# mims-harvard/GNNDelete

Hardware: AMD Instinct MI355X
Metric: Del-op train iters/sec (higher is better)
Workload: dtype f32; 1 GPU; synth-collab GCN 2-layer, 5.0% IN edge deletion, full-graph Del step (both_layerwise, mse_mean); num_nodes=235868, in_dim=128, hidden_dim=128, out_dim=64, train_edges_undirected=2122296, df_edges=53057, sdf_edges=1602188, spmm_nnz=1838056, S1=178921, S2=188697, hip_graph=True, matrix_products=fp32 matrix instruction (v_mfma_f32_32x32x2_f32), parallelism=single, ranks_seen=1

## Files before the change

### gnndelete_amd/_lib.py

```python
import ctypes
import os
import re

_HERE = os.path.dirname(os.path.abspath(__file__))
LIB_PATH = os.environ.get('GNNDELETE_HIP_LIB') or os.path.join(_HERE, 'lib', 'libgnndelete_hip.so')
HEADER_PATH = os.path.join(os.path.dirname(_HERE), 'include', 'gnndelete_hip.h')

_i32, _i64, _f32, _f64, _p = ctypes.c_int32, ctypes.c_int64, ctypes.c_float, ctypes.c_double, ctypes.c_void_p

ABI_VERSION = 9

PROTOTYPES = {
    'gd_abi_version': (ctypes.c_int, []),
    'gd_last_error_string': (ctypes.c_char_p, []),
    'gd_build_source_hash': (ctypes.c_char_p, []),
    'gd_matrix_split': (ctypes.c_int, []),
    'gd_set_matrix_split': (ctypes.c_int, [ctypes.c_int]),
    'gd_csr_from_coo_workspace': (_i64, [_i32, _i64]),
    'gd_csr_from_coo': (ctypes.c_int, [_p, _p, _i64, _i32, _p, _p, _p, _p, _p, _i64, _p]),
    'gd_gcn_norm_f32': (ctypes.c_int, [_p, _p, _i32, _p, _p]),
    'gd_spmm_csr_f32': (ctypes.c_int, [_p, _p, _p, _p, _i64, _p, _i64, _p, _f32, _i32, _i32, _p]),
    'gd_spmm_csr_balanced_f32': (ctypes.c_int, [_p, _i32, _p, _i32, _p, _p, _p, _i64, _p, _i64, _p, _f32, _p, _p, _i32,
                                                _i32, _i32, _p, _p]),
    'gd_spmm_csr_onepass_f32': (ctypes.c_int, [_p, _i32, _p, _p, _p, _i64, _p, _i64, _p, _f32, _p, _i32, _i32, _i32, _p, _p]),
    'gd_spmm_csr_onepass_wide_f32': (ctypes.c_int, [_p, _i32, _p, _p, _p, _i64, _p, _i64, _p, _f32, _p, _i32, _i32, _i32, _p, _p]),
    'gd_rows_gemm_wgrad_reduce_f32': (ctypes.c_int, [_p, _i32, _i32, _i32, _p, _i32, _p, _p, _p, _p, _f64, _f64, _f64, _f64, _p]),
    'gd_step_tail_f32': (ctypes.c_int, [_p, _i32, _i32, _i32, _p, _p, _p, _p, _p, _i32, _i32, _i32, _p, _p, _p, _p, _f64, _f64, _f64, _f64,
                                        _p, _i32, _p, _i32, _p, _i32, _p, _p, _p, _p]),
    'gd_step_tail_parts_f32': (ctypes.c_int, [_p, _i32, _i32, _i32, _p, _p, _p, _p, _p, _i32, _i32, _i32, _p, _p, _p, _p, _f64, _f64, _f64, _f64,
                                        _p, _i32, _p, _i32, _p, _i32, _p, _p, _p, _p]),
    'gd_rgcn_conv_f32': (ctypes.c_int, [_p, _p, _p, _p, _p, _p, _i64, _i32, _p, _i32, _i32, _p, _i64, _i32, _i32, _p]),
    'gd_rowpair_loss_f32': (ctypes.c_int, [_i32, _p, _i64, _p, _p, _i64, _p, _i32, _i32, _p, _p, _i64, _p]),
    'gd_random_walk': (ctypes.c_int, [_p, _p, _i32, _p, _i32, _i32, ctypes.c_uint64, _p, _p]),
    'gd_negative_edges': (ctypes.c_int, [_p, _i64, _i64, ctypes.c_uint64, _p, _i64, _p, _i64, _p]),
    'gd_rank_counts_f32': (ctypes.c_int, [_p, _i64, _p, _i64, _p, _p, _p]),
    'gd_subset_rank_workspace': (_i64, [_i64, _i64]),
    'gd_subset_rank_metrics': (ctypes.c_int, [_p, _p, _p, _p, _p, _i64, _i64, _i64, _i64, _i64, _p, _p, _p, _i64, _p]),
    'gd_rgcn_tile_kl': (ctypes.c_int32, [_i32, _i32, _i32, _i32]),
    'gd_rgcn_pack_weight_f32': (ctypes.c_int, [_p, _i32, _i32, _i32, _i32, _i32, _p, _p]),
    'gd_rgcn_wave_covers': (ctypes.c_int32, [_i32, _i32, _i32]),
    'gd_rgcn_wave_conv_f32': (ctypes.c_int, [_p, _i32, _i32, _p, _i32, _p, _p, _p, _p, _i64, _i32, _p, _i32, _p, _i64, _i32, _i32, _i32, _p]),
    'gd_rgcn_tile_conv_f32': (ctypes.c_int, [_p, _p, _p, _p, _p, _p, _p, _i32, _p, _i64, _i32, _p, _i32, _i32, _p, _i64, _i32,
                                             _i32, _p, _p, _i32, _p, _p]),
    'gd_rgcn_mean_f32': (ctypes.c_int, [_p, _p, _p, _i64, _p, _i64, _i32, _i32, _i32, _p]),
    'gd_gat_aggregate_f32': (ctypes.c_int, [_p, _p, _p, _p, _p, _i64, _p, _i64, _p, _p, _f32, _i32, _i32, _p]),
    'gd_gat_aggregate_bwd_f32': (ctypes.c_int, [_p, _p, _p, _p, _p, _p, _p, _p, _p, _i64, _p, _i64, _p, _i64,
                                                _p, _p, _p, _f32, _i32, _i32, _p]),
    'gd_gat_balanced_scratch': (_i64, [_i32, _i32]),
    'gd_gat_aggregate_balanced_f32': (ctypes.c_int, [_p, _i32, _p, _i32, _i32, _p, _p, _p, _p, _i64, _p, _i64, _p, _p, _p,
                                                     _p, _f32, _i32, _i32, _i32, _p]),
    'gd_gat_edge_grads_balanced_f32': (ctypes.c_int, [_p, _i32, _p, _i32, _p, _p, _p, _p, _p, _p, _i64, _p, _i64, _p,
                                                      _p, _p, _p, _f32, _i32, _i32, _p, _p]),
    'gd_row_dots_f32': (ctypes.c_int, [_p, _i64, _i32, _i32, _p, _p, _p, _p, _p]),
    'gd_gat_transpose_edges_f32': (ctypes.c_int, [_p, _p, _p, _i32, _p, _p, _p]),
    'gd_rank1_add2_f32': (ctypes.c_int, [_p, _i64, _i32, _i32, _p, _p, _p, _p, _p]),
    'gd_segment_sum_f32': (ctypes.c_int, [_p, _p, _p, _i32, _p, _p]),
    'gd_rows_gemm_f32': (ctypes.c_int, [_p, _i64, _p, _i32, _p, _i32, _i32, _i32, _p, _i32, _p, _i64, _p, _p]),
    'gd_rows_gather_gemm_f32': (ctypes.c_int, [_p, _i64, _i64, _p, _i32, _p, _i32, _i32, _p, _i32, _p, _i64, _p]),
    'gd_rows_gemm_wgrad_workspace': (_i64, [_i32, _i32, _i32]),
    'gd_rows_gemm_ws_covers': (ctypes.c_int, [_i32, _i32, _i32]),
    'gd_rows_gemm_accumulate_f32': (ctypes.c_int, [_p, _i64, _p, _i32, _p, _i32, _i32, _i32, _p, _i64, _p]),
    'gd_rows_gemm_select_f32': (ctypes.c_int, [_p, _p, _p, _i64, _p, _i32, _p, _i32, _i32, _i32, _p, _i32, _p, _i64, _p]),
    'gd_rows_gemm_dots_f32': (ctypes.c_int, [_p, _p, _p, _i64, _p, _i32, _i32, _i32, _p, _i32, _p, _i64, _p, _i32, _p, _p, _p, _p,
                                             _p]),
    'gd_rows_gemm_signs_f32': (ctypes.c_int, [_p, _i64, _p, _i32, _p, _i32, _i32, _i32, _p, _i32, _p, _i64, _p, _p, _p]),
    'gd_rows_gemm_gated_f32': (ctypes.c_int, [_p, _i64, _p, _i32, _p, _i32, _i32, _i32, _p, _p, _i64, _p]),
    'gd_gate_rows_f32': (ctypes.c_int, [_p, _i64, _p, _i32, _p, _i32, _p, _i64, _p]),
    'gd_rows_gemm_gated_rank1_f32': (ctypes.c_int, [_p, _i64, _p, _i32, _p, _i32, _i32, _i32, _p, _p, _p, _p, _p, _p, _i64, _p]),
    'gd_rows_gemm_wgrad_f32': (ctypes.c_int, [_p, _i64, _p, _p, _i64, _p, _p, _p, _i32, _i32, _i32, _p, _i32, _p, _p]),
    'gd_induced_subgraph_workspace': (_i64, [_i32]),
    'gd_induced_subgraph': (ctypes.c_int, [_p, _p, _p, _i32, _p, _i32, _p, _i32, _p, _i64, _p, _p, _p, _p, _p, _p, _p, _p, _p,
                                           _p, _i64, _p]),
    'gd_batch_csr_workspace': (_i64, [_i32, _i64]),
    'gd_batch_csr': (ctypes.c_int, [_p, _p, _i64, _i32, _i32, _p, _p, _p, _p, _p, _p, _p, _p, _i64, _p]),
    'gd_batch_loss_terms_workspace': (_i64, [_i32, _i64]),
    'gd_batch_loss_terms': (ctypes.c_int, [_p, _i64, _p, _i64, _i32, _p, _i32, _i32, _f32, _f32, _p, _p, _p, _p, _p, _i64, _p]),
    'gd_rowpair_mse_workspace': (_i64, [_i32]),
    'gd_rowpair_mse_f32': (ctypes.c_int, [_p, _i64, _p, _i64, _i32, _p, _p, _i32, _p, _p, _p, _p, _i64, _i32,
                                          _p, _p, _p]),
    'gd_rowtarget_mse_workspace': (_i64, [_i32]),
    'gd_rowtarget_mse_f32': (ctypes.c_int, [_p, _i64, _p, _i32, _p, _p, _p, _p, _i32, _p, _i64, _p, _p, _p]),
    'gd_rowtarget_mse_pair_covers': (ctypes.c_int32, [_i32, _i32]),
    'gd_rowtarget_mse_pair_f32': (ctypes.c_int, [_p, _i64, _p, _i32, _p, _p, _p, _p, _i32, _p, _i64, _p, _p, _i64, _p, _i32, _p, _p, _p, _p, _i32, _p, _i64, _p, _p]),
    'gd_gemm_f32_workspace': (_i64, [_i32, _i32, _i32]),
    'gd_gemm_f32': (ctypes.c_int, [_p, _i64, _p, _i32, _p, _i32, _i32, _p, _p, _i64, _p, _p]),
    'gd_edge_dot_f32': (ctypes.c_int, [_p, _i64, _i32, _p, _p, _p, _i64, _p, _i64, _p, _p]),
    'gd_edge_dot_bwd_f32': (ctypes.c_int, [_p, _i64, _i32, _p, _p, _p, _i64, _p, _p, _i64, _p, _i64, _p]),
    'gd_rows_gemm_wgrad_adam_f32': (ctypes.c_int, [_p, _i64, _p, _p, _i64, _p, _p, _p, _i32, _i32, _i32, _p, _i32, _p,
                                                   _p, _p, _p, _p, _f64, _f64, _f64, _f64, _p]),
    'gd_rows_gemm_wgrad_blocks': (_i32, [_i32]),
    'gd_rows_gemm_wgrad_loss_f32': (ctypes.c_int, [_p, _i64, _p, _p, _i64, _p, _p, _p, _p, _p, _p, _i32, _i32, _i32, _p, _i32,
                                                   _p, _p, _p, _p, _p, _p, _f64, _f64, _f64, _f64, _p]),
    'gd_del_loss_bwd_blocks': (_i32, [_i32]),
    'gd_del_loss_bwd_f32': (ctypes.c_int, [_p, _i64, _p, _i32, _p, _i32, _p, _p, _p, _p, _p, _i64, _p, _i64, _p, _p]),
    'gd_del_loss_bwd_wgrad_f32': (ctypes.c_int, [_p, _i64, _p, _i32, _p, _i32, _p, _p, _p, _p, _p, _i64, _p, _i64, _p, _p, _p]),
    'gd_del_loss_bwd_wgrad_parts': (ctypes.c_int32, [_i32, _i32]),
    'gd_del_loss_bwd_wgrad_parts_f32': (ctypes.c_int, [_p, _i64, _p, _i32, _p, _i32, _p, _p, _p, _p, _p, _i64, _p, _i64, _p, _p, _i32, _p]),
    'gd_del_loss_fold_wgrad_covers': (ctypes.c_int32, [_i32, _i32, _i32]),
    'gd_del_loss_fold_wgrad_parts_f32': (ctypes.c_int, [_p, _i64, _p, _i32, _p, _i32, _p, _p, _p, _p, _p, _i64, _p, _i32, _p, _p, _p, _i32, _p]),
    'gd_del1_loss_wgrad_covers': (ctypes.c_int32, [_i32, _i32]),
    'gd_del1_loss_wgrad_parts': (ctypes.c_int32, [_i32]),
    'gd_del1_chain_loss_wgrad_f32': (ctypes.c_int, [_p, _i64, _p, _i32, _p, _i32, _p, _i64, _p, _p, _p, _p, _p, _p, _i64, _i32, _p, _p, _p, _p, _p, _p, _p, _i32, _p]),
    'gd_del1_loss_wgrad_f32': (ctypes.c_int, [_p, _i64, _p, _i32, _p, _i32, _p, _i64, _p, _p, _p, _p, _p, _p, _i64, _p, _p, _i32, _p]),
    'gd_rowtarget_mse_blocks': (_i32, [_i32]),
    'gd_rowfold_loss_blocks': (_i32, [_i32]),
    'gd_rowfold_loss_f32': (ctypes.c_int, [_i32, _p, _i64, _p, _i32, _i32, _p, _p, _p, _p, _i32, _p, _i64, _p, _p]),
    'gd_rowfold_kld_scale_f32': (ctypes.c_int, [_p, _i32, _f32, _f32, _f32, _f32, _p, _p, _i32, _i32, _p, _i64, _p, _p]),
    'gd_loss_finalize_f32': (ctypes.c_int, [_p, _i32, _p, _i32, _p, _p, _i32, _p, _p, _p]),
    'gd_pairs_sigmoid_mse_workspace': (_i64, [_i32, _i32]),
    'gd_pairs_sigmoid_mse_f32': (ctypes.c_int, [_p, _i64, _p, _i32, _i32, _p, _i64, _f32, _p, _p, _p, _p]),
    'gd_edgeprob_dec_workspace': (_i64, [_i64, _i32]),
    'gd_edgeprob_dec_f32': (ctypes.c_int, [_p, _i64, _i64, _i32, _p, _i64, _p, _i64, _i64, _f32, _p, _p, _p, _p, _p, _p, _p]),
    'gd_edge_incidence_workspace': (_i64, [_i64, _i64]),
    'gd_edge_incidence': (ctypes.c_int, [_p, _p, _i64, _i64, _p, _p, _p, _p, _i64, _p]),
    'gd_edge_incidence_fixed_bytes': (_i64, [_i64, _i64]),
    'gd_edge_incidence_fixed': (ctypes.c_int, [_p, _p, _i64, _i64, _p, _i64, _p, _i64, _p]),
    'gd_edge_incidence_update_workspace': (_i64, [_i64, _i64]),
    'gd_edge_incidence_update': (ctypes.c_int, [_p, _p, _p, _i64, _i64, _i64, _p, _p, _p, _p, _i64, _p]),
    'gd_rows_add_f32': (ctypes.c_int, [_p, _i64, _i64, _p, _i32, _p, _i64, _f32, _i32, _p]),
    'gd_edgeprob_record_f32': (ctypes.c_int, [_p, _p, _f32, _f32, _p, _i32, _p, _p]),
    'gd_edgeprob_batch_loss_workspace': (_i64, [_i64, _i64, _i32]),
    'gd_edgeprob_batch_loss_f32': (ctypes.c_int, [_p, _i64, _i64, _p, _i64, _i64, _i32, _p, _i64, _p, _i64, _i64, _p, _p, _i64, _f32, _f32,
                                                  _p, _i64, _p, _p, _p, _p, _p, _p, _p, _i64, _p, _p]),
    'gd_edge_bce_workspace': (_i64, [_i64, _i32]),
    'gd_edge_bce_f32': (ctypes.c_int, [_p, _i64, _i64, _i32, _p, _i64, _i64, _p, _i64, _i64, _f32, _p, _p, _p, _p, _p, _p, _p]),
    'gd_col_sum_workspace': (_i64, [_i64, _i32]),
    'gd_col_sum_f32': (ctypes.c_int, [_p, _i64, _i64, _i32, _p, _p, _p, _p, _p, _p]),
    'gd_row_nll_workspace': (_i64, [_i64, _i32]),
    'gd_row_nll_f32': (ctypes.c_int, [_p, _i64, _i64, _i32, _i32, _p, _i64, _p, _f32, _p, _i64, _p, _p, _p]),
    'gd_adam_at_f32': (ctypes.c_int, [_p, _p, _p, _p, _p, _i64, _f64, _f64, _f64, _f64, _p]),
    'gd_adam_f32': (ctypes.c_int, [_p, _p, _p, _p, _p, _i64, _f64, _f64, _f64, _f64, _p]),
    'gd_segment_softmax_f32': (ctypes.c_int, [_p, _p, _i32, _p, _p]),
    'gd_segment_softmax_bwd_f32': (ctypes.c_int, [_p, _p, _p, _i32, _p, _p]),
    'gd_rowpair_dot_f32': (ctypes.c_int, [_p, _i64, _p, _p, _i64, _p, _i64, _i32, _p, _p]),
    'gd_spmm_csr_onepass_aux_f32': (ctypes.c_int, [_p, _i32, _p, _p, _p, _p, _i64, _p, _i64, _p, _i32, _i32, _i32, _p, _p]),
    'gd_typed_wgrad_f32': (ctypes.c_int, [_p, _i32, _p, _p, _p, _p, _i64, _p, _i64, _i32, _i32, _i32, _p, _p]),
    'gd_typed_edge_dot_f32': (ctypes.c_int, [_p, _p, _p, _i64, _p, _i64, _p, _i64, _p, _i32, _i32, _i32, _p, _p]),
    'gd_comm_unique_id': (ctypes.c_int, [_p]),
    'gd_comm_init': (ctypes.c_int, [_p, _i32, _i32, ctypes.POINTER(ctypes.c_void_p)]),
    'gd_comm_destroy': (ctypes.c_int, [_p]),
    'gd_allreduce_f32': (ctypes.c_int, [_p, _i64, _p, _p]),
    'gd_exchange_rows_f32': (ctypes.c_int, [_p, _p, _p, _p, _i32, _i32, _p, _p]),
}

_lib = None


class GnnDeleteHipError(RuntimeError):
    pass


def declared_symbols():
    with open(HEADER_PATH) as f:
        text = re.sub(r'/\*.*?\*/', '', f.read(), flags=re.S)
    return sorted(set(re.findall(r'\b(gd_[a-z0-9_]+)\s*\(', text)))


def _sources_hash():
    from .source_hash import source_files, source_hash
    return source_hash() if all(os.path.exists(f) for f in source_files()) and os.path.isdir(os.path.join(_HERE, 'csrc')) else None


def build_stamp():
    return lib().gd_build_source_hash().decode(), _sources_hash()


def lib():
    global _lib
    if _lib is None:
        if not os.path.exists(LIB_PATH):
            raise GnnDeleteHipError(
                f'{LIB_PATH} is missing: the HIP extension is not built. Run '
                '`python -c "import __graft_entry__ as g; g.build()"` (or `make -C gnndelete_amd/csrc`). '
                'There is no CPU fallback.')
        import torch
        handle = ctypes.CDLL(LIB_PATH)
        for name, (res, args) in PROTOTYPES.items():
            fn = getattr(handle, name)
            fn.restype, fn.argtypes = res, args
        if handle.gd_abi_version() != ABI_VERSION:
            raise GnnDeleteHipError(f'libgnndelete_hip.so ABI version {handle.gd_abi_version()}, this package binds version {ABI_VERSION}: rebuild (make -C gnndelete_amd/csrc)')
        built, here = handle.gd_build_source_hash().decode(), _sources_hash()
        if here is not None and built != here and not os.environ.get('GNNDELETE_HIP_LIB') and os.environ.get('GD_ALLOW_STALE_LIB') != '1':
            raise GnnDeleteHipError(f'{LIB_PATH} was built from other sources (stamp {built}, sources here {here}): run '
                                    '`make -C gnndelete_amd/csrc` (or set GD_ALLOW_STALE_LIB=1 to load it anyway)')
# ... 18 lines not shown
```

### gnndelete_amd/csrc/del_fused.hip

```cpp
#include <stdlib.h>

#include "common.h"

namespace gd {

using f32x16 = __attribute__((ext_vector_type(16))) float;

struct DelLoss {
  const int32_t* slot;
  const float* tm;
  const float* coef;
  const float* cnt_signed;
  float* partials;
};

template <int NT, bool WG>
__global__ __launch_bounds__(256, (NT == 2 && WG) ? 1 : 2) void del_loss_bwd_kernel(const float* __restrict__ p, int64_t ld_p,
                                                              const int32_t* __restrict__ idx, int32_t n_sel,
                                                              const float* __restrict__ w, DelLoss loss,
                                                              float* __restrict__ dz, int64_t ld_dz,
                                                              float* __restrict__ dp, int64_t ld_dp,
                                                              float* __restrict__ wg_partials) {
  constexpr int D = 32 * NT;
  constexpr int PB = D + 4;
// ... 497 lines not shown
#pragma unroll
      for (int i = 0; i < 8; ++i)
        *reinterpret_cast<float4*>(tp + r * PTP + kq * 32 + 4 * i) = make_float4(livef * x[i].x, livef * x[i].y, livef * x[i].z, livef * x[i].w);
      const float cf = ls_cur >= 0 ? cf_raw : 0.f, cn = ls_cur >= 0 ? cn_raw : 0.f;
      float sq = 0.f;
      uint32_t bits[2] = {0u, 0u};
      float* zrow = z + (int64_t)row * ld_z + cb + 4 * kq;
#pragma unroll
      for (int t = 0; t < 4; ++t) {
        const float4 zv = make_float4(acc[t][0], acc[t][1], acc[t][2], acc[t][3]);
        *reinterpret_cast<float4*>(zrow + 16 * t) = zv;
        bits[t >> 1] |= ((zv.x > 0.f ? 1u : 0u) | (zv.y > 0.f ? 2u : 0u) | (zv.z > 0.f ? 4u : 0u) | (zv.w > 0.f ? 8u : 0u)) << (16 * (t & 1) + 4 * kq);
        const float4 d4 = make_float4(zv.x - tv[t].x, zv.y - tv[t].y, zv.z - tv[t].z, zv.w - tv[t].w);
        sq = fmaf(d4.x, d4.x, sq); sq = fmaf(d4.y, d4.y, sq); sq = fmaf(d4.z, d4.z, sq); sq = fmaf(d4.w, d4.w, sq);
        float4 gv = make_float4(cf * d4.x, cf * d4.y, cf * d4.z, cf * d4.w);
        if (HAS_ADD) gv = f4_add(gv, av[t]);
        *reinterpret_cast<float4*>(tz + r * PTZ + 16 * t + 4 * kq) = gv;
      }
      sq *= livef;
      if (cn >= 0.f) ls0 = fmaf(cn, sq, ls0); else ls1 = fmaf(-cn, sq, ls1);
#pragma unroll
      for (int q = 0; q < 2; ++q) {
        bits[q] |= (uint32_t)__shfl_xor((int)bits[q], 16);
        bits[q] |= (uint32_t)__shfl_xor((int)bits[q], 32);
      }
      if (live && kq == 0) {
        sign_out[(int64_t)s_a * 4 + 2 * half + 0] = bits[0];
        sign_out[(int64_t)s_a * 4 + 2 * half + 1] = bits[1];
      }
      __builtin_amdgcn_sched_barrier(0);
      fetch_rows(row_n);
      fetch_targets(ls_n, row_n);
      __builtin_amdgcn_fence(__ATOMIC_ACQ_REL, "wavefront");
      __builtin_amdgcn_wave_barrier();
#pragma unroll
      for (int sp = 0; sp < 4; ++sp) {
        float a_op[8], b_op[4];
#pragma unroll
        for (int ta = 0; ta < 8; ++ta) a_op[ta] = tp[(4 * sp + kq) * PTP + 16 * ta + r];
#pragma unroll
        for (int tb = 0; tb < 4; ++tb) b_op[tb] = tz[(4 * sp + kq) * PTZ + 16 * tb + r];
#pragma unroll
        for (int ta = 0; ta < 8; ++ta)
#pragma unroll
          for (int tb = 0; tb < 4; ++tb)
            gacc[ta * 4 + tb] = __builtin_amdgcn_mfma_f32_16x16x4f32(a_op[ta], b_op[tb], gacc[ta * 4 + tb], 0, 0, 0);
      }
      __builtin_amdgcn_fence(__ATOMIC_ACQ_REL, "wavefront");
      __builtin_amdgcn_wave_barrier();
      __builtin_amdgcn_sched_barrier(0);
    }
  }
  __syncthreads();
  float* const red = wl;
#pragma unroll
  for (int ta = 0; ta < 8; ++ta)
#pragma unroll
    for (int tb = 0; tb < 4; ++tb)
#pragma unroll
      for (int v = 0; v < 4; ++v) red[wave * D * H + (16 * ta + 4 * kq + v) * H + 16 * tb + r] = gacc[ta * 4 + tb][v];
  __syncthreads();
  for (int slot = blockIdx.x; slot < n_part; slot += gridDim.x) {
    float* const out = wg_partials + (int64_t)slot * D * D;
    const bool mine = slot == (int)blockIdx.x;
    for (int e = tid; e < D * D; e += 256) {
      const int i = e >> 7, c = e & 127, hf = c >> 6, ch = c & 63;
      out[e] = mine ? red[hf * D * H + i * H + ch] + red[(2 + hf) * D * H + i * H + ch] : 0.f;
    }
  }
  ls0 = wave_sum(ls0);
  ls1 = wave_sum(ls1);
  if (lane == 0) { lred[0][wave] = ls0; lred[1][wave] = ls1; }
  __syncthreads();
  if (tid == 0) {
    for (int slot = blockIdx.x; slot < n_part; slot += gridDim.x) {
      const bool mine = slot == (int)blockIdx.x;
      loss.partials[2 * slot + 0] = mine ? (lred[0][0] + lred[0][1]) + (lred[0][2] + lred[0][3]) : 0.f;
      loss.partials[2 * slot + 1] = mine ? (lred[1][0] + lred[1][1]) + (lred[1][2] + lred[1][3]) : 0.f;
    }
  }
}

struct ChainRank1 { const float* ra; const float* ua; const float* rb; const float* ub; };
template <bool RANK1>
__global__ __launch_bounds__(256) __attribute__((amdgpu_waves_per_eu(1, 1))) void del1_chain_ws_kernel(
    const float* __restrict__ p, int64_t ld_p, const int32_t* __restrict__ idx, int32_t n_sel, const float* __restrict__ w,
    float* __restrict__ z, int64_t ld_z, uint32_t* __restrict__ sign_io, DelLoss loss, const float* __restrict__ dt, int64_t ld_dt,
    const float* __restrict__ w_next, float* __restrict__ wg_partials, int32_t n_part, ChainRank1 r1) {
  constexpr int D = 128, H = 64, PTP = 144, PTZ = 80;
  constexpr int kTiles = 4 * (16 * PTP + 16 * PTZ);
  extern __shared__ __attribute__((aligned(16))) float wl[];
  __shared__ float lred[2][4];
  const int tid = threadIdx.x, lane = tid & 63;
  const int wave = __builtin_amdgcn_readfirstlane(tid >> 6);
  const int half = wave & 1, pair = wave >> 1, cb = H * half;
  const int r = lane & 15, kq = lane >> 4;
  float* const tp = wl + wave * (16 * PTP + 16 * PTZ);
  float* const tz = tp + 16 * PTP;
  float4* const wimg = reinterpret_cast<float4*>(wl + kTiles);
  float4* const w2img = wimg + 2 * 4 * 8 * 64;
  {
    float4 fv[16];
#pragma unroll
    for (int it = 0; it < 16; ++it) {
      const int e = tid + 256 * it;
      const int ln = e & 63, i_ = (e >> 6) & 7, t_ = (e >> 9) & 3, h_ = e >> 11;
      const float* src = w + (int64_t)(16 * i_ + 4 * (ln >> 4)) * D + 64 * h_ + 16 * t_ + (ln & 15);
      fv[it] = make_float4(src[0], src[D], src[2 * D], src[3 * D]);
    }
#pragma unroll
    for (int it = 0; it < 16; ++it) wimg[tid + 256 * it] = fv[it];
#pragma unroll
    for (int it = 0; it < 8; ++it) {
      const int e = tid + 256 * it;
      const int ln = e & 63, i_ = (e >> 6) & 3, t_ = (e >> 8) & 3, h_ = e >> 10;
      const float* src = w_next + (int64_t)(16 * i_ + 4 * (ln >> 4)) * D + 64 * h_ + 16 * t_ + (ln & 15);
      fv[it] = make_float4(src[0], src[D], src[2 * D], src[3 * D]);
    }
#pragma unroll
    for (int it = 0; it < 8; ++it) w2img[tid + 256 * it] = fv[it];
  }
  __syncthreads();
  const float4* const wmine = wimg + (half * 4) * 8 * 64 + lane;
  const float4* const w2mine = w2img + (half * 4) * 4 * 64 + lane;
  const int n_units = (n_sel + 15) >> 4;
  const int n_pairs = gridDim.x * 2, pid = blockIdx.x * 2 + pair;
  const int u_lo = (int)((int64_t)n_units * pid / n_pairs), u_hi = (int)((int64_t)n_units * (pid + 1) / n_pairs);

  auto slot_of = [&](int u) -> int { return min(min(u, n_units - 1) * 16 + r, n_sel - 1); };
  int32_t row_n = idx[slot_of(u_lo)], ls_n = loss.slot[slot_of(u_lo)];
  int32_t row_nn = idx[slot_of(u_lo + 1)], ls_nn = loss.slot[slot_of(u_lo + 1)];
  __builtin_amdgcn_sched_barrier(0);
  f32x4w gacc[32];
#pragma unroll
  for (int i = 0; i < 32; ++i) gacc[i] = f32x4w{0.f, 0.f, 0.f, 0.f};
  float ls0 = 0.f, ls1 = 0.f;

  float4 x[8], dv[4], tv[4];
  float4 ua4[RANK1 ? 4 : 1], ub4[RANK1 ? 4 : 1];
  float ra_row = 0.f, rb_row = 0.f;
  if (RANK1) {
#pragma unroll
    for (int t = 0; t < 4; ++t) {
      ua4[t] = *reinterpret_cast<const float4*>(r1.ua + cb + 16 * t + 4 * kq);
      ub4[t] = *reinterpret_cast<const float4*>(r1.ub + cb + 16 * t + 4 * kq);
    }
  }
  uint2 old_bits;
  float cf_raw, cn_raw;
  int32_t ls_cur;
  auto fetch_targets = [&](int32_t u) {
    const int uc = max(u, 0);
    const float* trow = loss.tm + (int64_t)uc * D + cb + 4 * kq;
#pragma unroll
    for (int t = 0; t < 4; ++t) tv[t] = *reinterpret_cast<const float4*>(trow + 16 * t);
    cf_raw = loss.coef[uc];
    cn_raw = loss.cnt_signed[uc];
    ls_cur = u;
  };
  auto fetch_rows = [&](int32_t row, int u) {
    const float4* src = reinterpret_cast<const float4*>(p + (int64_t)row * ld_p + 4 * kq);
#pragma unroll
    for (int i = 0; i < 8; ++i) x[i] = src[4 * i];
    const float4* dsrc = reinterpret_cast<const float4*>(dt + (int64_t)row * ld_dt + 4 * kq);
#pragma unroll
    for (int i = 0; i < 4; ++i) dv[i] = dsrc[4 * i];
    old_bits = *reinterpret_cast<const uint2*>(sign_io + (int64_t)slot_of(u) * 4 + 2 * half);
    if (RANK1) { ra_row = r1.ra[row]; rb_row = r1.rb[row]; }
  };
  if (u_lo < u_hi) {
    fetch_rows(row_n, u_lo);
    fetch_targets(ls_n);
    for (int u = u_lo; u < u_hi; ++u) {
      const int32_t row = row_n;
      const int s_a = min(u, n_units - 1) * 16 + r;
      const bool live = s_a < n_sel;
      const float livef = live ? 1.f : 0.f;
      row_n = row_nn;
      ls_n = ls_nn;
      row_nn = idx[slot_of(u + 2)];
      ls_nn = loss.slot[slot_of(u + 2)];
      f32x4w acc[4], dacc[4];
      {
        float4 wq[2][4];
#pragma unroll
        for (int t = 0; t < 4; ++t) wq[0][t] = wmine[(t * 8) * 64];
#pragma unroll
        for (int i = 0; i < 8; ++i) {
          if (i + 1 < 8) {
#pragma unroll
            for (int t = 0; t < 4; ++t) wq[(i + 1) & 1][t] = wmine[(t * 8 + i + 1) * 64];
          }
          const float xv[4] = {x[i].x, x[i].y, x[i].z, x[i].w};
#pragma unroll
          for (int c = 0; c < 4; ++c)
#pragma unroll
            for (int t = 0; t < 4; ++t) {
              const float4 wf = wq[i & 1][t];
              const float wa = c == 0 ? wf.x : c == 1 ? wf.y : c == 2 ? wf.z : wf.w;
              if (i == 0 && c == 0) acc[t] = __builtin_amdgcn_mfma_f32_16x16x4f32(wa, xv[0], f32x4w{0.f, 0.f, 0.f, 0.f}, 0, 0, 0);
              else acc[t] = __builtin_amdgcn_mfma_f32_16x16x4f32(wa, xv[c], acc[t], 0, 0, 0);
            }
        }
#pragma unroll
        for (int t = 0; t < 4; ++t) wq[0][t] = w2mine[(t * 4) * 64];
#pragma unroll
        for (int i = 0; i < 4; ++i) {
          if (i + 1 < 4) {
#pragma unroll
            for (int t = 0; t < 4; ++t) wq[(i + 1) & 1][t] = w2mine[(t * 4 + i + 1) * 64];
          }
          const float xv[4] = {dv[i].x, dv[i].y, dv[i].z, dv[i].w};
#pragma unroll
          for (int c = 0; c < 4; ++c)
#pragma unroll
            for (int t = 0; t < 4; ++t) {
              const float4 wf = wq[i & 1][t];
              const float wa = c == 0 ? wf.x : c == 1 ? wf.y : c == 2 ? wf.z : wf.w;
              if (i == 0 && c == 0) dacc[t] = __builtin_amdgcn_mfma_f32_16x16x4f32(wa, xv[0], f32x4w{0.f, 0.f, 0.f, 0.f}, 0, 0, 0);
              else dacc[t] = __builtin_amdgcn_mfma_f32_16x16x4f32(wa, xv[c], dacc[t], 0, 0, 0);
            }
        }
      }
      __builtin_amdgcn_sched_barrier(0);
#pragma unroll
      for (int i = 0; i < 8; ++i)
        *reinterpret_cast<float4*>(tp + r * PTP + 16 * i + 4 * kq) = make_float4(livef * x[i].x, livef * x[i].y, livef * x[i].z, livef * x[i].w);
      const float cf = ls_cur >= 0 ? cf_raw : 0.f, cn = ls_cur >= 0 ? cn_raw : 0.f;
      float sq = 0.f;
      uint32_t bits[2] = {0u, 0u};
      const uint32_t ob[2] = {old_bits.x, old_bits.y};
      const float ra_c = ra_row, rb_c = rb_row;
      float* zrow = z + (int64_t)row * ld_z + cb + 4 * kq;
#pragma unroll
      for (int t = 0; t < 4; ++t) {
        const float4 zv = make_float4(acc[t][0], acc[t][1], acc[t][2], acc[t][3]);
        *reinterpret_cast<float4*>(zrow + 16 * t) = zv;
        bits[t >> 1] |= ((zv.x > 0.f ? 1u : 0u) | (zv.y > 0.f ? 2u : 0u) | (zv.z > 0.f ? 4u : 0u) | (zv.w > 0.f ? 8u : 0u)) << (16 * (t & 1) + 4 * kq);
        const float4 d4 = make_float4(zv.x - tv[t].x, zv.y - tv[t].y, zv.z - tv[t].z, zv.w - tv[t].w);
        sq = fmaf(d4.x, d4.x, sq); sq = fmaf(d4.y, d4.y, sq); sq = fmaf(d4.z, d4.z, sq); sq = fmaf(d4.w, d4.w, sq);
        const uint32_t m = ob[t >> 1] >> (16 * (t & 1) + 4 * kq);
        float4 dq = make_float4(dacc[t][0], dacc[t][1], dacc[t][2], dacc[t][3]);
        if (RANK1) {
          dq.x = fmaf(rb_c, ub4[t].x, fmaf(ra_c, ua4[t].x, dq.x)); dq.y = fmaf(rb_c, ub4[t].y, fmaf(ra_c, ua4[t].y, dq.y));
          dq.z = fmaf(rb_c, ub4[t].z, fmaf(ra_c, ua4[t].z, dq.z)); dq.w = fmaf(rb_c, ub4[t].w, fmaf(ra_c, ua4[t].w, dq.w));
        }
        const float4 gv = make_float4(cf * d4.x + ((m & 1u) ? dq.x : 0.f), cf * d4.y + ((m & 2u) ? dq.y : 0.f),
                                      cf * d4.z + ((m & 4u) ? dq.z : 0.f), cf * d4.w + ((m & 8u) ? dq.w : 0.f));
        *reinterpret_cast<float4*>(tz + r * PTZ + 16 * t + 4 * kq) = gv;
      }
      sq *= livef;
      if (cn >= 0.f) ls0 = fmaf(cn, sq, ls0); else ls1 = fmaf(-cn, sq, ls1);
#pragma unroll
      for (int q = 0; q < 2; ++q) {
        bits[q] |= (uint32_t)__shfl_xor((int)bits[q], 16);
        bits[q] |= (uint32_t)__shfl_xor((int)bits[q], 32);
      }
      if (live && kq == 0) *reinterpret_cast<uint2*>(sign_io + (int64_t)s_a * 4 + 2 * half) = make_uint2(bits[0], bits[1]);
      __builtin_amdgcn_sched_barrier(0);
      fetch_rows(row_n, u + 1);
      fetch_targets(ls_n);
      __builtin_amdgcn_fence(__ATOMIC_ACQ_REL, "wavefront");
      __builtin_amdgcn_wave_barrier();
#pragma unroll
      for (int sp = 0; sp < 4; ++sp) {
        float a_op[8], b_op[4];
#pragma unroll
        for (int ta = 0; ta < 8; ++ta) a_op[ta] = tp[(4 * sp + kq) * PTP + 16 * ta + r];
#pragma unroll
        for (int tb = 0; tb < 4; ++tb) b_op[tb] = tz[(4 * sp + kq) * PTZ + 16 * tb + r];
#pragma unroll
        for (int ta = 0; ta < 8; ++ta)
#pragma unroll
          for (int tb = 0; tb < 4; ++tb)
            gacc[ta * 4 + tb] = __builtin_amdgcn_mfma_f32_16x16x4f32(a_op[ta], b_op[tb], gacc[ta * 4 + tb], 0, 0, 0);
      }
      __builtin_amdgcn_fence(__ATOMIC_ACQ_REL, "wavefront");
      __builtin_amdgcn_wave_barrier();
      __builtin_amdgcn_sched_barrier(0);
    }
  }
  __syncthreads();
  float* const red = wl;
#pragma unroll
  for (int ta = 0; ta < 8; ++ta)
#pragma unroll
    for (int tb = 0; tb < 4; ++tb)
#pragma unroll
      for (int v = 0; v < 4; ++v) red[wave * D * H + (16 * ta + 4 * kq + v) * H + 16 * tb + r] = gacc[ta * 4 + tb][v];
  __syncthreads();
  for (int slot = blockIdx.x; slot < n_part; slot += gridDim.x) {
    float* const out = wg_partials + (int64_t)slot * D * D;
    const bool mine = slot == (int)blockIdx.x;
    for (int e = tid; e < D * D; e += 256) {
      const int i = e >> 7, c = e & 127, hf = c >> 6, ch = c & 63;
      out[e] = mine ? red[hf * D * H + i * H + ch] + red[(2 + hf) * D * H + i * H + ch] : 0.f;
    }
  }
  ls0 = wave_sum(ls0);
  ls1 = wave_sum(ls1);
  if (lane == 0) { lred[0][wave] = ls0; lred[1][wave] = ls1; }
  __syncthreads();
  if (tid == 0) {
    for (int slot = blockIdx.x; slot < n_part; slot += gridDim.x) {
      const bool mine = slot == (int)blockIdx.x;
      loss.partials[2 * slot + 0] = mine ? (lred[0][0] + lred[0][1]) + (lred[0][2] + lred[0][3]) : 0.f;
      loss.partials[2 * slot + 1] = mine ? (lred[1][0] + lred[1][1]) + (lred[1][2] + lred[1][3]) : 0.f;
    }
  }
}

static inline int del_fused_grid(int32_t n_sel) {
  const int n_tiles = (n_sel + 31) / 32;
  int grid = (n_tiles + 3) / 4;
  if (grid > 1024) grid = 1024;
  return grid < 1 ? 1 : grid;
}

}

extern "C" int32_t gd_del_loss_bwd_blocks(int32_t n_sel) { return n_sel > 0 ? gd::del_fused_grid(n_sel) : 0; }

extern "C" int32_t gd_rows_gemm_wgrad_blocks(int32_t n_sel);

static int del_loss_bwd_impl(const float* p, int64_t ld_p, const int32_t* idx, int32_t n_sel, const float* w,
                             int32_t d, const int32_t* loss_slot, const float* tm, const float* coef,
                             const float* cnt_signed, float* dz, int64_t ld_dz, float* dp, int64_t ld_dp,
                             float* loss_partials, float* wgrad_partials, bool with_wgrad, void* stream, int32_t n_part_req = 0) {
  using namespace gd;
  const char* name = with_wgrad ? "gd_del_loss_bwd_wgrad_f32" : "gd_del_loss_bwd_f32";
  if (n_sel == 0) return GD_OK;
  GD_REQUIRE(p && idx && w && loss_slot && tm && coef && cnt_signed && dp && loss_partials && (with_wgrad ? wgrad_partials != nullptr : dz != nullptr),
             GD_E_NULL, "%s: null pointer", name);
  GD_REQUIRE(d == 32 || d == 64, GD_E_DIM, "%s: d=%d must be 32 or 64", name, d);
  GD_REQUIRE(ld_p >= d && (!dz || ld_dz >= d) && ld_dp >= d && ld_p % 4 == 0 && (!dz || ld_dz % 4 == 0) && ld_dp % 4 == 0, GD_E_DIM,
             "%s: bad row strides", name);
  GD_REQUIRE(aligned16(p) && aligned16(tm) && (!dz || aligned16(dz)) && aligned16(dp) && (!with_wgrad || aligned16(wgrad_partials)), GD_E_ALIGN,
             "%s: unaligned", name);
  GD_REQUIRE(p != dp && p != dz && dz != dp, GD_E_DIM, "%s: buffers must not alias", name);
  hipStream_t s = (hipStream_t)stream;
  const DelLoss loss{loss_slot, tm, coef, cnt_signed, loss_partials};
  if (!with_wgrad) {
    const dim3 grid(del_fused_grid(n_sel));
    const size_t lds = ((size_t)d * d + (size_t)d * (d + 4)) * sizeof(float);
    switch (d / 32) {
      case 1: hipLaunchKernelGGL((del_loss_bwd_kernel<1, false>), grid, dim3(256), lds, s, p, ld_p, idx, n_sel, w, loss, dz, ld_dz, dp, ld_dp, nullptr); break;
      default: hipLaunchKernelGGL((del_loss_bwd_kernel<2, false>), grid, dim3(256), lds, s, p, ld_p, idx, n_sel, w, loss, dz, ld_dz, dp, ld_dp, nullptr); break;
    }
    return launched("del_loss_bwd");
  }
  static const bool ws_on = [] { const char* e = getenv("GD_DEL2_WS"); return !(e && atoi(e) == 0); }();
  if (ws_on && d == 64 && n_sel >= 65536) {
    const int n_all = gd_rows_gemm_wgrad_blocks(n_sel);
    const int n_part = n_part_req > 0 ? n_part_req : n_all;
    GD_REQUIRE(n_part <= n_all && n_part >= (ws_cu_count() < n_all ? ws_cu_count() : n_all), GD_E_DIM,
               "%s: n_part=%d outside [gd_del_loss_bwd_wgrad_parts, gd_rows_gemm_wgrad_blocks = %d]", name, n_part, n_all);
    const int grid_ws = ws_cu_count() < n_part ? ws_cu_count() : n_part;
    constexpr int kLdsWs = 4 * 64 * 64 * 4;
    if (dz) {
      static const hipError_t a1 = hipFuncSetAttribute(reinterpret_cast<const void*>(&del_loss_bwd_ws_kernel<true>), hipFuncAttributeMaxDynamicSharedMemorySize, kLdsWs);
      if (a1 != hipSuccess) return fail(-(int)a1, "gd_del_loss_bwd_wgrad_f32: %s", hipGetErrorString(a1));
      hipLaunchKernelGGL((del_loss_bwd_ws_kernel<true>), dim3(grid_ws), dim3(256), kLdsWs, s, p, ld_p, idx, n_sel, w, loss, dz, ld_dz, dp, ld_dp,
                         wgrad_partials, n_part, DelFold{nullptr, nullptr});
    } else {
      static const hipError_t a0 = hipFuncSetAttribute(reinterpret_cast<const void*>(&del_loss_bwd_ws_kernel<false>), hipFuncAttributeMaxDynamicSharedMemorySize, kLdsWs);
      if (a0 != hipSuccess) return fail(-(int)a0, "gd_del_loss_bwd_wgrad_f32: %s", hipGetErrorString(a0));
      hipLaunchKernelGGL((del_loss_bwd_ws_kernel<false>), dim3(grid_ws), dim3(256), kLdsWs, s, p, ld_p, idx, n_sel, w, loss, dz, ld_dz, dp, ld_dp,
                         wgrad_partials, n_part, DelFold{nullptr, nullptr});
    }
    return launched("del_loss_bwd_ws");
  }
  GD_REQUIRE(n_part_req == 0 || n_part_req == gd_rows_gemm_wgrad_blocks(n_sel), GD_E_DIM,
             "%s: n_part=%d but this size leaves gd_rows_gemm_wgrad_blocks(n_sel) = %d partials", name, n_part_req, gd_rows_gemm_wgrad_blocks(n_sel));
  const dim3 grid(gd_rows_gemm_wgrad_blocks(n_sel));
#define GD_DF_CASE(NT_)                                                                                                        \
  do {                                                                                                                         \
    constexpr int kD = 32 * NT_;                                                                                               \
    constexpr int kLds = (kD * kD + kD * (kD + 4) + 4 * 32 * (kD + 4)) * 4;                                                    \
    static_assert(kLds >= 4 * kD * kD * 4, "block sum needs 4 D^2 floats");                                                    \
// ... 68 lines not shown
  static const hipError_t at = hipFuncSetAttribute(reinterpret_cast<const void*>(&del_loss_bwd_ws_kernel<false, true>), hipFuncAttributeMaxDynamicSharedMemorySize, kLdsWs);
  if (at != hipSuccess) return fail(-(int)at, "%s: %s", name, hipGetErrorString(at));
  const DelLoss loss{loss_slot, tm, coef, cnt_signed, loss_partials};
  hipLaunchKernelGGL((del_loss_bwd_ws_kernel<false, true>), dim3(grid_ws), dim3(256), kLdsWs, (hipStream_t)stream, p, ld_p, idx, n_sel, w, loss,
                     static_cast<float*>(nullptr), (int64_t)0, g, ld_g, wgrad_partials, n_part, DelFold{w_next, w_fold});
  return launched("del_loss_fold_ws");
}

extern "C" int32_t gd_del1_loss_wgrad_covers(int32_t n_sel, int32_t d) {
  static const bool on = [] { const char* e = getenv("GD_DEL1_FUSED"); return !(e && atoi(e) == 0); }();
  return on && d == 128 && n_sel >= 65536 ? 1 : 0;
}

extern "C" int32_t gd_del1_loss_wgrad_parts(int32_t n_sel) {
  if (n_sel <= 0) return 0;
  const int nb = gd_rows_gemm_wgrad_blocks(n_sel);
  return gd::ws_cu_count() < nb ? gd::ws_cu_count() : nb;
}

extern "C" int gd_del1_loss_wgrad_f32(const float* p, int64_t ld_p, const int32_t* idx, int32_t n_sel, const float* w, int32_t d,
                                      float* z, int64_t ld_z, uint32_t* sign_out, const int32_t* loss_slot, const float* tm,
                                      const float* coef, const float* cnt_signed, const float* g_add, int64_t ld_gadd,
                                      float* loss_partials, float* wgrad_partials, int32_t n_part, void* stream) {
  using namespace gd;
  const char* name = "gd_del1_loss_wgrad_f32";
  if (n_sel == 0) return GD_OK;
  GD_REQUIRE(p && idx && w && z && sign_out && loss_slot && tm && coef && cnt_signed && loss_partials && wgrad_partials, GD_E_NULL,
             "%s: null pointer", name);
  GD_REQUIRE(d == 128, GD_E_DIM, "%s: d=%d must be 128 (other widths: gd_rows_gemm_signs_f32 + gd_rows_gemm_wgrad_loss_f32)", name, d);
  GD_REQUIRE(ld_p >= d && ld_z >= d && ld_p % 4 == 0 && ld_z % 4 == 0 && (!g_add || (ld_gadd >= d && ld_gadd % 4 == 0)), GD_E_DIM,
             "%s: bad row strides", name);
  GD_REQUIRE(aligned16(p) && aligned16(z) && aligned16(tm) && aligned16(w) && (!g_add || aligned16(g_add)) && aligned16(wgrad_partials),
             GD_E_ALIGN, "%s: unaligned", name);
  GD_REQUIRE(p != z && g_add != z, GD_E_DIM, "%s: z must not alias p or g_add (the two waves of a pair read whole rows)", name);
  hipStream_t s = (hipStream_t)stream;
  const DelLoss loss{loss_slot, tm, coef, cnt_signed, loss_partials};
  GD_REQUIRE(n_part >= 1 && n_part <= gd_rows_gemm_wgrad_blocks(n_sel), GD_E_DIM,
             "%s: n_part=%d outside [1, gd_rows_gemm_wgrad_blocks(n_sel)=%d]", name, n_part, gd_rows_gemm_wgrad_blocks(n_sel));
  const int grid = ws_cu_count() < n_part ? ws_cu_count() : n_part;
  constexpr int kLds = 4 * 128 * 64 * 4;
  if (g_add) {
    static const hipError_t a1 = hipFuncSetAttribute(reinterpret_cast<const void*>(&del1_loss_wgrad_ws_kernel<true>), hipFuncAttributeMaxDynamicSharedMemorySize, kLds);
    if (a1 != hipSuccess) return fail(-(int)a1, "%s: %s", name, hipGetErrorString(a1));
    hipLaunchKernelGGL((del1_loss_wgrad_ws_kernel<true>), dim3(grid), dim3(256), kLds, s, p, ld_p, idx, n_sel, w, z, ld_z, sign_out, loss, g_add,
                       ld_gadd, wgrad_partials, n_part);
  } else {
    static const hipError_t a0 = hipFuncSetAttribute(reinterpret_cast<const void*>(&del1_loss_wgrad_ws_kernel<false>), hipFuncAttributeMaxDynamicSharedMemorySize, kLds);
    if (a0 != hipSuccess) return fail(-(int)a0, "%s: %s", name, hipGetErrorString(a0));
    hipLaunchKernelGGL((del1_loss_wgrad_ws_kernel<false>), dim3(grid), dim3(256), kLds, s, p, ld_p, idx, n_sel, w, z, ld_z, sign_out, loss, nullptr,
                       0, wgrad_partials, n_part);
  }
  return launched("del1_loss_wgrad_ws");
}

extern "C" int gd_del1_chain_loss_wgrad_f32(const float* p, int64_t ld_p, const int32_t* idx, int32_t n_sel, const float* w, int32_t d,
                                            float* z, int64_t ld_z, uint32_t* sign_io, const int32_t* loss_slot, const float* tm,
                                            const float* coef, const float* cnt_signed, const float* dt, int64_t ld_dt, int32_t d_next,
                                            const float* w_next, const float* row_a, const float* col_a, const float* row_b,
                                            const float* col_b, float* loss_partials, float* wgrad_partials, int32_t n_part,
                                            void* stream) {
  using namespace gd;
  const char* name = "gd_del1_chain_loss_wgrad_f32";
  if (n_sel == 0) return GD_OK;
  GD_REQUIRE(p && idx && w && z && sign_io && loss_slot && tm && coef && cnt_signed && dt && w_next && loss_partials && wgrad_partials, GD_E_NULL,
             "%s: null pointer", name);
  GD_REQUIRE(d == 128 && d_next == 64, GD_E_DIM, "%s: widths %d / %d must be 128 / 64", name, d, d_next);
  GD_REQUIRE(ld_p >= d && ld_z >= d && ld_dt >= d_next && ld_p % 4 == 0 && ld_z % 4 == 0 && ld_dt % 4 == 0, GD_E_DIM, "%s: bad row strides", name);
  GD_REQUIRE(aligned16(p) && aligned16(z) && aligned16(tm) && aligned16(dt) && aligned16(wgrad_partials) && (reinterpret_cast<uintptr_t>(sign_io) & 7u) == 0,
             GD_E_ALIGN, "%s: unaligned", name);
  GD_REQUIRE(p != z && dt != z, GD_E_DIM, "%s: z must not alias p or dt", name);
  GD_REQUIRE(n_part >= 1 && n_part <= gd_rows_gemm_wgrad_blocks(n_sel), GD_E_DIM,
             "%s: n_part=%d outside [1, gd_rows_gemm_wgrad_blocks(n_sel)=%d]", name, n_part, gd_rows_gemm_wgrad_blocks(n_sel));
  const DelLoss loss{loss_slot, tm, coef, cnt_signed, loss_partials};
  const int grid = ws_cu_count() < n_part ? ws_cu_count() : n_part;
  constexpr int kLds = (4 * (16 * 144 + 16 * 80) + 128 * 128 + 64 * 128) * 4;
  const bool rank1 = row_a || col_a || row_b || col_b;
  GD_REQUIRE(!rank1 || (row_a && col_a && row_b && col_b && aligned16(col_a) && aligned16(col_b)), GD_E_NULL,
             "%s: the rank-1 terms come as four pointers (row_a, col_a, row_b, col_b; 16-byte aligned column vectors)", name);
  const ChainRank1 r1{row_a, col_a, row_b, col_b};
  if (rank1) {
    static const hipError_t at = hipFuncSetAttribute(reinterpret_cast<const void*>(&del1_chain_ws_kernel<true>), hipFuncAttributeMaxDynamicSharedMemorySize, kLds);
    if (at != hipSuccess) return fail(-(int)at, "%s: %s", name, hipGetErrorString(at));
    hipLaunchKernelGGL(del1_chain_ws_kernel<true>, dim3(grid), dim3(256), kLds, (hipStream_t)stream, p, ld_p, idx, n_sel, w, z, ld_z, sign_io, loss, dt,
                       ld_dt, w_next, wgrad_partials, n_part, r1);
  } else {
    static const hipError_t at = hipFuncSetAttribute(reinterpret_cast<const void*>(&del1_chain_ws_kernel<false>), hipFuncAttributeMaxDynamicSharedMemorySize, kLds);
    if (at != hipSuccess) return fail(-(int)at, "%s: %s", name, hipGetErrorString(at));
    hipLaunchKernelGGL(del1_chain_ws_kernel<false>, dim3(grid), dim3(256), kLds, (hipStream_t)stream, p, ld_p, idx, n_sel, w, z, ld_z, sign_io, loss, dt,
                       ld_dt, w_next, wgrad_partials, n_part, r1);
  }
  return launched("del1_chain_ws");
}
```

### gnndelete_amd/csrc/rows_gemm.hip

```cpp
#include "common.h"

namespace gd {

using f32x16 = __attribute__((ext_vector_type(16))) float;
using bf16x8 = __attribute__((ext_vector_type(8))) __bf16;
using bf16x2 = __attribute__((ext_vector_type(2))) __bf16;
using f32x2 = __attribute__((ext_vector_type(2))) float;
using u32x4v = __attribute__((ext_vector_type(4))) uint32_t;

__device__ inline void split8(const float4 a, const float4 b, bf16x8 (&s)[3]) {
  const f32x2 v[4] = {{a.x, a.y}, {a.z, a.w}, {b.x, b.y}, {b.z, b.w}};
  u32x4v p[3];
#pragma unroll
  for (int i = 0; i < 4; ++i) {
    f32x2 r = v[i];
#pragma unroll
    for (int q = 0; q < 3; ++q) {
      const uint32_t w = __builtin_bit_cast(uint32_t, __builtin_convertvector(r, bf16x2));
      p[q][i] = w;
      if (q < 2) {
        f32x2 h;
        h[0] = __builtin_bit_cast(float, w << 16);
        h[1] = __builtin_bit_cast(float, w & 0xffff0000u);
        r = r - h;
// ... 567 lines not shown
  }
}

__global__ __launch_bounds__(256) void wgrad_reduce_kernel(const float* __restrict__ partials, int32_t n_part,
                                                           int32_t n_elem, int32_t accumulate,
                                                           float* __restrict__ dw) {
  __shared__ float4 red[16][16];
  const int v = threadIdx.x & 15, slice = threadIdx.x >> 4;
  const int e4 = blockIdx.x * 16 + v;
  const int n4 = n_elem >> 2;
  float4 s0 = f4_zero(), s1 = f4_zero(), s2 = f4_zero(), s3 = f4_zero();
  if (e4 < n4) {
    int b = slice;
    for (; b + 48 < n_part; b += 64) {
      const float4 p0 = reinterpret_cast<const float4*>(partials + (int64_t)b * n_elem)[e4];
      const float4 p1 = reinterpret_cast<const float4*>(partials + (int64_t)(b + 16) * n_elem)[e4];
      const float4 p2 = reinterpret_cast<const float4*>(partials + (int64_t)(b + 32) * n_elem)[e4];
      const float4 p3 = reinterpret_cast<const float4*>(partials + (int64_t)(b + 48) * n_elem)[e4];
      s0 = f4_add(s0, p0); s1 = f4_add(s1, p1); s2 = f4_add(s2, p2); s3 = f4_add(s3, p3);
    }
    for (; b < n_part; b += 16) s0 = f4_add(s0, reinterpret_cast<const float4*>(partials + (int64_t)b * n_elem)[e4]);
  }
  red[slice][v] = f4_add(f4_add(s0, s1), f4_add(s2, s3));
  __syncthreads();
  if (slice == 0 && e4 < n4) {
    float4 t = accumulate ? reinterpret_cast<float4*>(dw)[e4] : f4_zero();
#pragma unroll
    for (int i = 0; i < 16; ++i) t = f4_add(t, red[i][v]);
    reinterpret_cast<float4*>(dw)[e4] = t;
  }
}

__global__ __launch_bounds__(256) void wgrad_reduce_adam_kernel(const float* __restrict__ partials, int32_t n_part,
                                                                int32_t n_elem, int32_t accumulate,
                                                                float* __restrict__ dw, float* __restrict__ param,
                                                                float* __restrict__ m, float* __restrict__ v,
                                                                const int32_t* __restrict__ iter, double lr, double beta1,
                                                                double beta2, double eps) {
  __shared__ float4 red[16][16];
  const int vv = threadIdx.x & 15, slice = threadIdx.x >> 4;
  const int e4 = blockIdx.x * 16 + vv;
  const int n4 = n_elem >> 2;
  float4 s0 = f4_zero(), s1 = f4_zero(), s2 = f4_zero(), s3 = f4_zero();
  if (e4 < n4) {
    int b = slice;
    for (; b + 48 < n_part; b += 64) {
      const float4 p0 = reinterpret_cast<const float4*>(partials + (int64_t)b * n_elem)[e4];
      const float4 p1 = reinterpret_cast<const float4*>(partials + (int64_t)(b + 16) * n_elem)[e4];
      const float4 p2 = reinterpret_cast<const float4*>(partials + (int64_t)(b + 32) * n_elem)[e4];
      const float4 p3 = reinterpret_cast<const float4*>(partials + (int64_t)(b + 48) * n_elem)[e4];
      s0 = f4_add(s0, p0); s1 = f4_add(s1, p1); s2 = f4_add(s2, p2); s3 = f4_add(s3, p3);
    }
    for (; b < n_part; b += 16) s0 = f4_add(s0, reinterpret_cast<const float4*>(partials + (int64_t)b * n_elem)[e4]);
  }
  red[slice][vv] = f4_add(f4_add(s0, s1), f4_add(s2, s3));
  __syncthreads();
  if (slice == 0 && e4 < n4) {
    float4 t4 = accumulate ? reinterpret_cast<float4*>(dw)[e4] : f4_zero();
#pragma unroll
    for (int i = 0; i < 16; ++i) t4 = f4_add(t4, red[i][vv]);
    reinterpret_cast<float4*>(dw)[e4] = t4;
    const AdamScalars sc = adam_scalars(lr, beta1, beta2, eps, *iter + 1);
    float4 p4 = reinterpret_cast<float4*>(param)[e4], m4 = reinterpret_cast<float4*>(m)[e4],
           v4 = reinterpret_cast<float4*>(v)[e4];
    adam_update(p4.x, m4.x, v4.x, t4.x, sc);
    adam_update(p4.y, m4.y, v4.y, t4.y, sc);
    adam_update(p4.z, m4.z, v4.z, t4.z, sc);
    adam_update(p4.w, m4.w, v4.w, t4.w, sc);
    reinterpret_cast<float4*>(param)[e4] = p4;
    reinterpret_cast<float4*>(m)[e4] = m4;
    reinterpret_cast<float4*>(v)[e4] = v4;
  }
}

struct TailJob {
  const float* partials; int32_t n_part, n_elem, accumulate;
  float* dw; float* param; float* m; float* v;
};
struct TailFin {
  const float* p1; int32_t n1; const float* p2; int32_t n2;
  float* hist; int32_t capacity; int32_t* pos; int32_t* iter; int32_t* arrive;
};

__global__ __launch_bounds__(256) void step_tail_kernel(TailJob j1, TailJob j2, TailFin fin, double lr, double beta1, double beta2,
                                                        double eps) {
  __shared__ float4 red[16][16];
  __shared__ float fred[4][256];
  __shared__ int32_t t_sh;
  const int nb1 = (j1.n_elem / 4 + 15) / 16, nb2 = (j2.n_elem / 4 + 15) / 16;
  const int tid = threadIdx.x;
  if ((int)blockIdx.x < nb1 + nb2) {
    const bool first = (int)blockIdx.x < nb1;
    const TailJob j = first ? j1 : j2;
    const int blk = first ? blockIdx.x : blockIdx.x - nb1;
    if (tid == 0) {
      int32_t t = atomicAdd(fin.iter, 0);
      asm volatile("" : "+v"(t));
      atomicAdd(fin.arrive + (t < 0 ? 1 : 0), 1);
      t_sh = t + 1;
    }
    const int vv = tid & 15, slice = tid >> 4;
    const int e4 = blk * 16 + vv;
    const int n4 = j.n_elem >> 2;
    float4 s0 = f4_zero(), s1 = f4_zero(), s2 = f4_zero(), s3 = f4_zero();
    if (e4 < n4) {
      int b = slice;
      for (; b + 48 < j.n_part; b += 64) {
        const float4 p0 = reinterpret_cast<const float4*>(j.partials + (int64_t)b * j.n_elem)[e4];
        const float4 p1 = reinterpret_cast<const float4*>(j.partials + (int64_t)(b + 16) * j.n_elem)[e4];
        const float4 p2 = reinterpret_cast<const float4*>(j.partials + (int64_t)(b + 32) * j.n_elem)[e4];
        const float4 p3 = reinterpret_cast<const float4*>(j.partials + (int64_t)(b + 48) * j.n_elem)[e4];
        s0 = f4_add(s0, p0); s1 = f4_add(s1, p1); s2 = f4_add(s2, p2); s3 = f4_add(s3, p3);
      }
      for (; b < j.n_part; b += 16) s0 = f4_add(s0, reinterpret_cast<const float4*>(j.partials + (int64_t)b * j.n_elem)[e4]);
    }
    red[slice][vv] = f4_add(f4_add(s0, s1), f4_add(s2, s3));
    __syncthreads();
    if (slice == 0 && e4 < n4) {
      float4 t4 = j.accumulate ? reinterpret_cast<float4*>(j.dw)[e4] : f4_zero();
#pragma unroll
      for (int i = 0; i < 16; ++i) t4 = f4_add(t4, red[i][vv]);
      reinterpret_cast<float4*>(j.dw)[e4] = t4;
      const AdamScalars sc = adam_scalars(lr, beta1, beta2, eps, t_sh);
      float4 p4 = reinterpret_cast<float4*>(j.param)[e4], m4 = reinterpret_cast<float4*>(j.m)[e4],
             v4 = reinterpret_cast<float4*>(j.v)[e4];
      adam_update(p4.x, m4.x, v4.x, t4.x, sc);
      adam_update(p4.y, m4.y, v4.y, t4.y, sc);
      adam_update(p4.z, m4.z, v4.z, t4.z, sc);
      adam_update(p4.w, m4.w, v4.w, t4.w, sc);
      reinterpret_cast<float4*>(j.param)[e4] = p4;
      reinterpret_cast<float4*>(j.m)[e4] = m4;
      reinterpret_cast<float4*>(j.v)[e4] = v4;
    }
    return;
  }
  float a = 0.f, b = 0.f, c = 0.f, d = 0.f;
  for (int i = tid; i < fin.n1; i += 256) { a += fin.p1[2 * i]; b += fin.p1[2 * i + 1]; }
  for (int i = tid; i < fin.n2; i += 256) { c += fin.p2[2 * i]; d += fin.p2[2 * i + 1]; }
  fred[0][tid] = a; fred[1][tid] = b; fred[2][tid] = c; fred[3][tid] = d;
  __syncthreads();
  for (int off = 128; off > 0; off >>= 1) {
    if (tid < off) {
#pragma unroll
      for (int q = 0; q < 4; ++q) fred[q][tid] += fred[q][tid + off];
    }
    __syncthreads();
  }
  if (tid < 4) fin.hist[(int64_t)(*fin.pos) * 4 + tid] = fred[tid][0];
  __syncthreads();
  if (tid == 0) {
    while (atomicAdd(fin.arrive, 0) < nb1 + nb2) __builtin_amdgcn_s_sleep(8);
    *fin.arrive = 0;
    *fin.pos = (*fin.pos + 1) % fin.capacity;
    atomicAdd(fin.iter, 1);
  }
}

__global__ __launch_bounds__(256) void wgrad_reduce_scalar_kernel(const float* __restrict__ partials, int32_t n_part,
                                                                  int32_t n_elem, int32_t accumulate,
                                                                  float* __restrict__ dw) {
  const int e = blockIdx.x * 256 + threadIdx.x;
  if (e >= n_elem) return;
  float s = accumulate ? dw[e] : 0.f;
  for (int b = 0; b < n_part; ++b) s += partials[(int64_t)b * n_elem + e];
  dw[e] = s;
}

static inline void wgrad_geometry(int32_t n_sel, int* n_blocks, int* rows_per_block) {
  int nb = (n_sel + 127) / 128;
  if (nb > 512) nb = 512;
  if (nb < (n_sel + kWgradMaxRows - 1) / kWgradMaxRows) nb = (n_sel + kWgradMaxRows - 1) / kWgradMaxRows;
  if (nb < 1) nb = 1;
  int rpb = (n_sel + nb - 1) / nb;
  rpb = (rpb + 31) / 32 * 32;
  if (rpb < 32) rpb = 32;
  *n_blocks = (n_sel + rpb - 1) / rpb;
  if (*n_blocks < 1) *n_blocks = 1;
  *rows_per_block = rpb;
}

}

static int rows_gemm_impl(const float* in, int64_t ld_in, const int32_t* idx, int32_t n_sel, const float* w,
                          int32_t d_in, int32_t d_out, int32_t trans_w, const float* bias, int32_t relu_in,
                          const uint32_t* gate_bits, uint32_t* sign_out, float* out, int64_t ld_out,
                          float* save_in, void* stream, const float* in_alt = nullptr, const uint8_t* sel = nullptr,
                          gd::RowDots dots = gd::RowDots{nullptr, nullptr, nullptr, nullptr}, const int64_t* gidx = nullptr,
                          int32_t n_in = 0) {
  using namespace gd;
  GD_REQUIRE(!sel || (in_alt && aligned16(in_alt) && in_alt != out && !gate_bits && !sign_out), GD_E_NULL,
             "gd_rows_gemm_select_f32: bad in_alt");
  GD_REQUIRE(in && w && out, GD_E_NULL, "gd_rows_gemm_f32: null pointer");
  GD_REQUIRE(n_sel >= 0 && d_in > 0 && d_out > 0 && ld_in >= d_in && ld_out >= d_out, GD_E_DIM,
             "gd_rows_gemm_f32: bad dims n_sel=%d d_in=%d d_out=%d", n_sel, d_in, d_out);
  GD_REQUIRE(in != out || d_in == d_out, GD_E_DIM, "gd_rows_gemm_f32: in-place needs d_in == d_out");
  GD_REQUIRE(!(gate_bits && sign_out), GD_E_DIM, "gd_rows_gemm_f32: gate and sign output are exclusive");
  if (n_sel == 0) return GD_OK;
  if (!gidx) {
    const int rc = rows_gemm_ws_try(in, ld_in, idx, n_sel, w, d_in, d_out, trans_w, bias, relu_in, gate_bits, sign_out, out, ld_out,
                                    save_in, stream, in_alt, sel, dots.u1, dots.u2, dots.o1, dots.o2);
    if (rc != 1) return rc;
  }
  hipStream_t s = (hipStream_t)stream;
  size_t lds = (size_t)d_in * 32 * (d_out / 32 == 3 ? 4 : d_out / 32) * sizeof(float);
  const int np = matrix_split();
  const bool mfma_ok = (d_out % 32 == 0) && d_out <= 128 && (d_in % 32 == 0) && lds <= 64 * 1024 && aligned16(in) &&
                       (ld_in % 4 == 0) && (!save_in || aligned16(save_in)) && aligned16(out) && (ld_out % 4 == 0) &&
                       (!bias || aligned16(bias));
  if (mfma_ok) {
    const int n_tiles = (n_sel + 31) / 32;
    int grid = (n_tiles + 7) / 8;
    static const int grid_cap = [] { const char* e = getenv("GD_ROWS_GEMM_GRID"); return e && atoi(e) > 0 ? atoi(e) : 512; }();
    if (grid > grid_cap) grid = grid_cap;
    static const bool spread_on = [] { const char* e = getenv("GD_ROWS_GEMM_SPREAD"); return !(e && atoi(e) == 0); }();
    if (spread_on && grid < ws_cu_count()) grid = n_tiles < ws_cu_count() ? n_tiles : ws_cu_count();
    const int kc_split = (np && (d_in == 64 || d_in == 128) && d_out >= 96) ? d_in / 32 : 0;
    const bool narrow_split = np && !kc_split && d_out == 64 && d_in == 128;
    if (kc_split || narrow_split) {
      lds = (size_t)3 * d_in * d_out * 2;
      if (grid > grid_cap / 2 && lds > 80 * 1024) grid = grid_cap / 2;
    }
    static const bool queue_on = [] { const char* e = getenv("GD_ROWS_GEMM_QUEUE"); return !(e && atoi(e) == 0); }();
    const bool use_queue = queue_on && !kc_split && !narrow_split && n_tiles >= 16 * 256 && !gidx;
    if (use_queue && grid > ws_cu_count()) grid = ws_cu_count();
#define GD_RG_KERNEL(NT, MODE, SELV, NPV, KCV, GV)                                                                 \
  do {                                                                                                            \
    if (use_queue && !NPV && !GV) {                                                                                 \
      auto kq = rows_gemm_mfma_kernel<NT, MODE, SELV, 0, 0, true>;                                                \
              \
      static const hipError_t onceq = hipFuncSetAttribute((const void*)kq, hipFuncAttributeMaxDynamicSharedMemorySize, 64 * 1024 + 64); \
      GD_REQUIRE(onceq == hipSuccess, -(int)onceq, "gd_rows_gemm_f32: cannot raise the LDS limit of the tile-queue kernel"); \
      hipLaunchKernelGGL(kq, dim3(grid), dim3(1024), lds, s, in, ld_in, idx, n_sel, w, d_in, trans_w,             \
                         bias, relu_in, out, ld_out, save_in, gate_bits, sign_out, in_alt, sel, dots, gidx, n_in); \
      break;                                                                                                      \
    }                                                                                                             \
    auto kern = rows_gemm_mfma_kernel<NT, MODE, SELV, NPV, KCV, false, GV>;                                            \
    if (NPV && lds > 64 * 1024) {                                                                                 \
      static const hipError_t once = hipFuncSetAttribute((const void*)kern, hipFuncAttributeMaxDynamicSharedMemorySize, 160 * 1024); \
// ... 199 lines not shown
  return gd_adam_at_f32(adam->param, dw, adam->m, adam->v, adam->iter, n_elem, adam->lr, adam->beta1, adam->beta2,
                        adam->eps, stream);
}

extern "C" int gd_rows_gemm_wgrad_f32(const float* a, int64_t ld_a, const int32_t* a_idx, const float* g, int64_t ld_g,
                                      const int32_t* g_idx, const float* relu_mask, const float* g_add,
                                      int32_t n_sel, int32_t d_a, int32_t d_b, float* dw, int32_t accumulate,
                                      float* partials, void* stream) {
  return wgrad_impl(nullptr, a, ld_a, a_idx, g, ld_g, g_idx, relu_mask, g_add, n_sel, d_a, d_b, dw, accumulate,
                    partials, nullptr, stream);
}

extern "C" int gd_rows_gemm_wgrad_adam_f32(const float* a, int64_t ld_a, const int32_t* a_idx, const float* g,
                                           int64_t ld_g, const int32_t* g_idx, const float* relu_mask,
                                           const float* g_add, int32_t n_sel, int32_t d_a, int32_t d_b, float* dw,
                                           int32_t accumulate, float* partials,
                                           float* param, float* exp_avg, float* exp_avg_sq, const int32_t* iter,
                                           double lr, double beta1, double beta2, double eps, void* stream) {
  GD_REQUIRE(param && exp_avg && exp_avg_sq && iter, GD_E_NULL, "gd_rows_gemm_wgrad_adam_f32: null optimizer state");
  const gd::AdamArgs adam{param, exp_avg, exp_avg_sq, iter, lr, beta1, beta2, eps};
  return wgrad_impl(nullptr, a, ld_a, a_idx, g, ld_g, g_idx, relu_mask, g_add, n_sel, d_a, d_b, dw, accumulate,
                    partials, &adam, stream);
}

extern "C" int gd_rows_gemm_wgrad_reduce_f32(const float* partials, int32_t n_sel, int32_t d_a, int32_t d_b, float* dw,
                                             int32_t accumulate, float* param, float* exp_avg, float* exp_avg_sq,
                                             const int32_t* iter, double lr, double beta1, double beta2, double eps,
                                             void* stream) {
  GD_REQUIRE(partials && dw, GD_E_NULL, "gd_rows_gemm_wgrad_reduce_f32: null pointer");
  GD_REQUIRE(!param || (exp_avg && exp_avg_sq && iter), GD_E_NULL, "gd_rows_gemm_wgrad_reduce_f32: null optimizer state");
  GD_REQUIRE(n_sel >= 0 && d_a > 0 && d_b > 0, GD_E_DIM, "gd_rows_gemm_wgrad_reduce_f32: bad dims");
  const gd::AdamArgs adam{param, exp_avg, exp_avg_sq, iter, lr, beta1, beta2, eps};
  return wgrad_impl(nullptr, nullptr, d_a, nullptr, nullptr, d_b, nullptr, nullptr, nullptr, n_sel, d_a, d_b, dw, accumulate,
                    const_cast<float*>(partials), param ? &adam : nullptr, stream, true);
}

static int step_tail_impl(const char* name, const float* partials1, int32_t nb1, int32_t d1, int32_t accumulate1, float* dw1, float* param1,
                          float* exp_avg1, float* exp_avg_sq1, const float* partials2, int32_t nb2, int32_t d2, int32_t accumulate2,
                          float* dw2, float* param2, float* exp_avg2, float* exp_avg_sq2, double lr, double beta1, double beta2,
                          double eps, const float* loss_partials1, int32_t n1, const float* loss_partials2, int32_t n2, float* hist,
                          int32_t capacity, int32_t* pos, int32_t* iter, int32_t* arrive, void* stream) {
  using namespace gd;
  GD_REQUIRE(partials1 && dw1 && param1 && exp_avg1 && exp_avg_sq1 && partials2 && dw2 && param2 && exp_avg2 && exp_avg_sq2, GD_E_NULL,
             "%s: null weight-gradient / optimizer pointer", name);
  GD_REQUIRE(hist && pos && iter && arrive && capacity > 0 && (n1 == 0 || loss_partials1) && (n2 == 0 || loss_partials2), GD_E_NULL,
             "%s: null bookkeeping pointer", name);
  GD_REQUIRE(nb1 > 0 && nb2 > 0 && d1 > 0 && d2 > 0 && (d1 * d1) % 4 == 0 && (d2 * d2) % 4 == 0, GD_E_DIM,
             "%s: both Del weights need rows and widths that are multiples of 2", name);
  GD_REQUIRE(aligned16(partials1) && aligned16(dw1) && aligned16(partials2) && aligned16(dw2), GD_E_ALIGN, "%s: unaligned", name);
  const TailJob j1{partials1, nb1, d1 * d1, accumulate1, dw1, param1, exp_avg1, exp_avg_sq1};
  const TailJob j2{partials2, nb2, d2 * d2, accumulate2, dw2, param2, exp_avg2, exp_avg_sq2};
  const TailFin fin{loss_partials1, n1, loss_partials2, n2, hist, capacity, pos, iter, arrive};
  const int grid = (j1.n_elem / 4 + 15) / 16 + (j2.n_elem / 4 + 15) / 16 + 1;
  GD_REQUIRE(grid <= 1024, GD_E_DIM, "%s: Del weights too large for the co-resident grid (%d blocks)", name, grid);
  hipLaunchKernelGGL(step_tail_kernel, dim3(grid), dim3(256), 0, (hipStream_t)stream, j1, j2, fin, lr, beta1, beta2, eps);
  return launched("step_tail");
}

extern "C" int gd_step_tail_f32(const float* partials1, int32_t n_sel1, int32_t d1, int32_t accumulate1, float* dw1, float* param1,
                                float* exp_avg1, float* exp_avg_sq1, const float* partials2, int32_t n_sel2, int32_t d2,
                                int32_t accumulate2, float* dw2, float* param2, float* exp_avg2, float* exp_avg_sq2, double lr,
                                double beta1, double beta2, double eps, const float* loss_partials1, int32_t n1,
                                const float* loss_partials2, int32_t n2, float* hist, int32_t capacity, int32_t* pos, int32_t* iter,
                                int32_t* arrive, void* stream) {
  int nb1 = 0, nb2 = 0, rpb;
  if (n_sel1 > 0) gd::wgrad_geometry(n_sel1, &nb1, &rpb);
  if (n_sel2 > 0) gd::wgrad_geometry(n_sel2, &nb2, &rpb);
  return step_tail_impl("gd_step_tail_f32", partials1, nb1, d1, accumulate1, dw1, param1, exp_avg1, exp_avg_sq1, partials2, nb2, d2, accumulate2,
                        dw2, param2, exp_avg2, exp_avg_sq2, lr, beta1, beta2, eps, loss_partials1, n1, loss_partials2, n2, hist, capacity,
                        pos, iter, arrive, stream);
}

extern "C" int gd_step_tail_parts_f32(const float* partials1, int32_t n_part1, int32_t d1, int32_t accumulate1, float* dw1, float* param1,
                                      float* exp_avg1, float* exp_avg_sq1, const float* partials2, int32_t n_part2, int32_t d2,
                                      int32_t accumulate2, float* dw2, float* param2, float* exp_avg2, float* exp_avg_sq2, double lr,
                                      double beta1, double beta2, double eps, const float* loss_partials1, int32_t n1,
                                      const float* loss_partials2, int32_t n2, float* hist, int32_t capacity, int32_t* pos,
                                      int32_t* iter, int32_t* arrive, void* stream) {
  return step_tail_impl("gd_step_tail_parts_f32", partials1, n_part1, d1, accumulate1, dw1, param1, exp_avg1, exp_avg_sq1, partials2, n_part2, d2,
                        accumulate2, dw2, param2, exp_avg2, exp_avg_sq2, lr, beta1, beta2, eps, loss_partials1, n1, loss_partials2, n2,
                        hist, capacity, pos, iter, arrive, stream);
}

extern "C" int32_t gd_rows_gemm_wgrad_blocks(int32_t n_sel) {
  int nb, rpb;
  gd::wgrad_geometry(n_sel, &nb, &rpb);
  return n_sel > 0 ? nb : 0;
}

extern "C" int gd_rows_gemm_wgrad_loss_f32(const float* a, int64_t ld_a, const int32_t* a_idx, const float* z,
                                           int64_t ld_z, const int32_t* z_idx, const int32_t* loss_slot,
                                           const float* tm, const float* coef, const float* cnt_signed,
                                           const float* g_add, int32_t n_sel, int32_t d_a, int32_t d_b, float* dw,
                                           int32_t accumulate, float* partials, float* loss_partials, float* param,
                                           float* exp_avg, float* exp_avg_sq, const int32_t* iter, double lr,
                                           double beta1, double beta2, double eps, void* stream) {
  GD_REQUIRE(n_sel == 0 || (loss_slot && tm && coef && cnt_signed), GD_E_NULL, "gd_rows_gemm_wgrad_loss_f32: null loss terms");
  GD_REQUIRE(loss_partials, GD_E_NULL, "gd_rows_gemm_wgrad_loss_f32: null loss_partials");
  GD_REQUIRE(!param || (exp_avg && exp_avg_sq && iter), GD_E_NULL, "gd_rows_gemm_wgrad_loss_f32: null optimizer state");
  GD_REQUIRE(n_sel == 0 || gd::aligned16(tm), GD_E_ALIGN, "gd_rows_gemm_wgrad_loss_f32: unaligned targets");
  const gd::WgradLoss loss{loss_slot, tm, coef, cnt_signed, loss_partials};
  const gd::AdamArgs adam{param, exp_avg, exp_avg_sq, iter, lr, beta1, beta2, eps};
  return wgrad_impl(&loss, a, ld_a, a_idx, z, ld_z, z_idx, nullptr, g_add, n_sel, d_a, d_b, dw, accumulate, partials,
                    param ? &adam : nullptr, stream);
}

namespace gd {
__global__ __launch_bounds__(256) void gate_rows_kernel(const float* __restrict__ src, int64_t ld_src, const int32_t* __restrict__ idx,
                                                        int32_t n_sel, const uint32_t* __restrict__ bits, int32_t d4, int32_t n_words,
                                                        float* __restrict__ out, int64_t ld_out) {
  const int64_t e = (int64_t)blockIdx.x * 256 + threadIdx.x;
  if (e >= (int64_t)n_sel * d4) return;
  const int s = (int)(e / d4), c4 = (int)(e % d4);
  const int64_t row = idx ? idx[s] : s;
  const uint32_t m = bits[(int64_t)s * n_words + (c4 >> 3)] >> (4 * (c4 & 7));
  float4 v = reinterpret_cast<const float4*>(src + row * ld_src)[c4];
  v.x = (m & 1u) ? v.x : 0.f; v.y = (m & 2u) ? v.y : 0.f; v.z = (m & 4u) ? v.z : 0.f; v.w = (m & 8u) ? v.w : 0.f;
  reinterpret_cast<float4*>(out + row * ld_out)[c4] = v;
}
}

extern "C" int gd_gate_rows_f32(const float* src, int64_t ld_src, const int32_t* idx, int32_t n_sel, const uint32_t* gate_bits,
                                int32_t d, float* out, int64_t ld_out, void* stream) {
  using namespace gd;
  GD_REQUIRE(src && gate_bits && out, GD_E_NULL, "gd_gate_rows_f32: null pointer");
  GD_REQUIRE(n_sel >= 0 && d > 0 && d % 4 == 0 && ld_src >= d && ld_out >= d && ld_src % 4 == 0 && ld_out % 4 == 0, GD_E_DIM,
             "gd_gate_rows_f32: d and the row pitches must be multiples of 4 (d=%d)", d);
  GD_REQUIRE(aligned16(src) && aligned16(out), GD_E_ALIGN, "gd_gate_rows_f32: unaligned pointer");
  if (n_sel == 0) return GD_OK;
  const int64_t total = (int64_t)n_sel * (d / 4);
  hipLaunchKernelGGL(gate_rows_kernel, dim3((unsigned)((total + 255) / 256)), dim3(256), 0, (hipStream_t)stream, src, ld_src, idx,
                     n_sel, gate_bits, d / 4, (d + 31) / 32, out, ld_out);
  return launched("gate_rows");
}
```

### gnndelete_amd/engine.py

```python
import os
import warnings
from typing import NamedTuple

import torch

from . import _lib, ops
from ._lib import check, ptr, stream_ptr
from .capture import capture_iterations
from .graph import graph_for
from .nn import GATConv, GCNConv, GINConv, RGCNConv, SAGEConv

LOSS_TYPES = ('both_all', 'both_layerwise', 'only2_layerwise', 'only2_all', 'only1')


class StepFacts(NamedTuple):
    mode: str
    loss_type: str
    family: str
    h: int
    o: int
    s1: int
    s2: int
    folded1: bool
    n_rows1: int
# ... 17 lines not shown
    cache_split: bool = True
    no_fused_loss1: bool = False
    no_step_tail: bool = False
    tail_fused_only: bool = False
    no_fused_wgrad2: bool = False
    del1_chain: bool = True
    no_gat_rank1_epilogue: bool = False
    no_loss_pair: bool = False
    no_gat_dots: bool = False
    rgcn_reorder: bool = True
    rgcn_node_major: bool = False
    rgcn_relu_pass: bool = False
    sage_root_in_spmm: bool = False
    pad_out: int = 64


def read_knobs(env=None):
    env = os.environ if env is None else env
    val = {}
    for name, default in Knobs._field_defaults.items():
        raw = env.get('GD_' + name.upper())
        if name == 'pad_out':
            try:
                val[name] = default if raw is None else int(raw)
            except ValueError:
                warnings.warn(f'GD_PAD_OUT={raw!r} is not an integer: the class dimension is not padded')
                val[name] = 0
        else:
            val[name] = (raw != '0') if default else (raw == '1')
    return Knobs(**val)


class StepForms(NamedTuple):
    split1: bool
    split2: bool
    out1: bool
    out2: bool
    fuse_loss1: bool
    fuse_l2: bool
    tail: bool
    fuse_wg2: bool
    fuse_del1: bool
    chain1: bool
    out_pair: bool
    rows_only: bool
    rgcn_rows_only: bool
    gat_dots: bool


def plan_step(facts, k):
    (mode, loss_type, family, h, o, s1, s2, folded1, n_rows1, inside1, folded2, n_rows2, inside2, cache_layer1, rows_only_asked,
     closed, w2_mfma, gin_ok, del1_covers, pair_covers) = facts
    mse = family == 'mse'
    mixed_ok = folded1 and folded2 and not k.no_split_loss and not k.no_split
    out2 = not inside2 and mixed_ok and mse and s2 > 0 and o in (32, 64) and n_rows2 > 0 and not k.no_fused_l2
    split2 = (inside2 or out2) and not k.no_split
    fuse_l2 = mse and split2 and folded1 and o in (32, 64) and n_rows2 > 0 and not k.no_fused_l2
    split1 = (not cache_layer1 or k.cache_split) and inside1 and not k.no_split
    loss1_ok = (mse and folded1 and folded2 and loss_type in ('both_layerwise', 'both_all', 'only1') and s1 > 0
                and h in (32, 64, 128) and n_rows1 > 0 and not k.no_fused_loss1)
    out1 = loss1_ok and not inside1 and mixed_ok
    fuse_loss1 = loss1_ok and (inside1 or out1)
    tail = (folded1 and folded2 and s1 > 0 and s2 > 0 and loss_type in ('both_layerwise', 'both_all') and h % 2 == 0 and o % 2 == 0
            and not k.no_step_tail
            and ((fuse_loss1 and fuse_l2) or (h in (32, 64, 128) and o in (32, 64, 128) and not k.tail_fused_only)))
    fuse_wg2 = tail and fuse_l2 and not k.no_fused_wgrad2
    fuse_del1 = tail and fuse_loss1 and split1 and loss_type in ('both_layerwise', 'only1') and del1_covers
    chain1 = (fuse_del1 and loss_type == 'both_layerwise' and h == 128 and o == 64 and k.del1_chain
              and (mode in ('gcn', 'gin') or (mode == 'gat' and w2_mfma and not k.no_gat_rank1_epilogue)))
    out_pair = out1 and out2 and fuse_loss1 and fuse_l2 and loss_type != 'only2_all' and pair_covers and not k.no_loss_pair
    rows_only = (rows_only_asked and (mode in ('gcn', 'gat', 'sage') or gin_ok) and split2 and s2 > 0
                 and not out1 and not out2 and closed)
    return StepForms(split1, split2, out1, out2, fuse_loss1, fuse_l2, tail, fuse_wg2, fuse_del1, chain1, out_pair, rows_only,
                     rows_only_asked and mode == 'rgcn', not k.no_gat_dots)


def read_del2_fold(env=None):
    env = os.environ if env is None else env
    return env.get('GD_DEL2_FOLD') != '0'


def plan_del2_fold(facts, forms, covers, enabled=True):
    return bool(enabled and covers and forms.chain1 and facts.mode in ('gcn', 'gin') and forms.fuse_wg2 and not forms.out2)


def _loss_coefficients(loss_type, alpha):
    if loss_type in ('both_all', 'both_layerwise', 'only2_layerwise'):
        return alpha, 1.0 - alpha
    return alpha, 1.0


LOSS_FAMILIES = {'mse_mean': ('mse', 'mean'), 'mse_sum': ('mse', 'sum'), 'kld_mean': ('kld', 'mean'), 'kld_sum': ('kld', 'sum'),
                 'cosine_mean': ('cosine', 'mean'), 'cosine_sum': ('cosine', 'sum')}
_ROWFOLD_FAMILY = {'cosine': 0, 'kld': 1}


def fold_row_terms(family, z_ori, rows, tgt, kind, d_valid=None):
    assert family in ('kld', 'cosine'), family
    d = z_ori.shape[1]
    dv = d if d_valid is None else int(d_valid)
    device = z_ori.device
    uniq, inv, c = torch.unique(rows, return_inverse=True, return_counts=True)
    kind_u = torch.zeros(uniq.numel(), dtype=torch.int32, device=device)
    kind_u[inv] = kind.to(torch.int32)
    if uniq.numel() == 0:
        return uniq, torch.zeros(0, d, dtype=torch.float64, device=device), c, kind_u, [0.0, 0.0]
    order = torch.argsort(inv, stable=True)
    o64 = z_ori[tgt[order]][:, :dv].double()
    if family == 'cosine':
        u = o64 / o64.norm(dim=1, keepdim=True).clamp_(min=1e-8)
        tm = torch.segment_reduce(u, 'sum', lengths=c, axis=0)
        k_row = torch.zeros(uniq.numel(), dtype=torch.float64, device=device)
    else:
        t = torch.softmax(o64, 1)
        tm = torch.segment_reduce(t, 'sum', lengths=c, axis=0)
        ent = torch.segment_reduce(torch.special.xlogy(t, t).sum(1), 'sum', lengths=c, axis=0)
        k_row = (ent - torch.special.xlogy(tm, tm / c[:, None].double()).sum(1)).clamp_(min=0.0)
    if dv < d:
        tm = torch.nn.functional.pad(tm, (0, d - dv))
    return uniq, tm, c, kind_u, [float(k_row[kind_u == 0].sum()), float(k_row[kind_u == 1].sum())]


def logged_loss(family, raw_sum, k_const, n):
    v = (raw_sum + k_const) / n
    return 1.0 - torch.exp(-v) if family == 'kld' else v


def _members(idx, n_sel, rows):
    pos = torch.searchsorted(idx, rows)
    return (pos < n_sel) & (idx[pos.clamp(max=n_sel - 1)] == rows), pos


class _LayerTerms:

    def __init__(self, pos_edge, neg_edge, ni_mask, z_ori, coef_r, coef_l, reduction, row_range=None, d_norm=None, family='mse'):
        device = z_ori.device
        self.family = family
        self.d_valid = z_ori.shape[1] if d_norm is None else int(d_norm)
        d = z_ori.shape[1]
        dn = d if d_norm is None else int(d_norm)
        pos, neg = pos_edge.to(device).long(), neg_edge.to(device).long()
        ni_rows = ni_mask.to(device).nonzero().flatten()
        m = pos.shape[1]
        if family != 'mse':
            dn = 1
        self.n_r = (2 * m * dn) if reduction == 'mean' else 1
        self.n_l = (ni_rows.numel() * dn) if reduction == 'mean' else 1
        self.count_r, self.count_l = 2 * m, int(ni_rows.numel())
        w_r, w_l = coef_r / max(self.n_r, 1), coef_l / max(self.n_l, 1)
        rows = torch.cat([pos[0], pos[1], ni_rows])
        tgt = torch.cat([neg[0], neg[1], ni_rows])
        kind = torch.cat([torch.zeros(2 * m, dtype=torch.int32, device=device),
                          torch.ones(ni_rows.numel(), dtype=torch.int32, device=device)])
        mixed = bool(ni_mask.to(device)[pos.flatten()].any()) if m else False
        if row_range is not None:
            mine = (rows >= row_range[0]) & (rows < row_range[1])
            rows, tgt, kind = rows[mine], tgt[mine], kind[mine]
        self.k_const = [0.0, 0.0]
        self.folded = not mixed
        if family != 'mse':
            if mixed:
                raise ValueError(f'the folded {family} loss needs one kind of term per row: a Neighborhood-Influence row of this request is an '
                                 'endpoint of a deleted edge (the autograd loop handles such a request)')
            if row_range is not None:
                raise ValueError(f'the folded {family} loss has no row-partitioned form (its scalar would need an all-reduce in mid-step)')
            uniq, tm, c, kind_u, self.k_const = fold_row_terms(family, z_ori, rows, tgt, kind, self.d_valid)
# ... 268 lines not shown
        self.uses_l1 = loss_type in ('both_all', 'both_layerwise', 'only1')
        self.uses_l2 = loss_type != 'only1'
        self.needs_l2_to_w1 = loss_type in ('both_all', 'both_layerwise', 'only2_all')

        f32 = dict(dtype=torch.float32, device=dev)
        self._mode = {GCNConv: 'gcn', GINConv: 'gin', GATConv: 'gat', SAGEConv: 'sage', RGCNConv: 'rgcn'}[type(conv2)]
        self.graph = None
        if self._mode != 'rgcn':
            self.graph = graph_for(edge_index, n, {'gcn': 'gcn', 'gin': 'sum', 'gat': 'gat', 'sage': 'mean'}[self._mode])
        w2 = {'gcn': lambda: conv2.lin.weight, 'gin': lambda: conv2.nn.weight, 'gat': lambda: conv2.lin_src.weight,
              'sage': lambda: conv2.lin_l.weight, 'rgcn': lambda: None}[self._mode]()
        rows_only_asked = bool(affected_rows_only)
        self.facts = StepFacts(
            mode=self._mode, loss_type=loss_type, family=self.family, h=self.h, o=self.o, s1=self.s1, s2=self.s2,
            folded1=self.t1.folded, n_rows1=self.t1.n_rows if self.t1.folded else 0, inside1=_rows_inside(self.t1, self.idx1, self.s1),
            folded2=self.t2.folded, n_rows2=self.t2.n_rows if self.t2.folded else 0, inside2=_rows_inside(self.t2, self.idx2, self.s2),
            cache_layer1=bool(cache_layer1), rows_only_asked=rows_only_asked,
            closed=rows_only_asked and self._mode != 'rgcn' and self.s2 > 0 and self._affected_rows_closed(),
            w2_mfma=w2 is not None and self._mfma_weight(w2),
            gin_ok=(self._mode == 'gin' and conv1.nn.out_features <= conv1.nn.in_features
                    and conv2.nn.out_features <= conv2.nn.in_features),
            del1_covers=bool(_lib.lib().gd_del1_loss_wgrad_covers(self.s1, self.h)),
            pair_covers=bool(_lib.lib().gd_rowtarget_mse_pair_covers(self.h, self.o)))
        self.forms = plan_step(self.facts, knobs)
        for name, on in self.forms._asdict().items():
            setattr(self, '_' + name, on)
        lib = _lib.lib()
        if self._out2:
            self.t2.order_inside_first(self.idx2, self.s2)
        if self._out1:
            self.t1.order_inside_first(self.idx1, self.s1)
        self.z1 = torch.empty(n, self.h, **f32)
        self.z2 = torch.empty(n, self.o, **f32)
        self.p2 = torch.empty(n, self.o, **f32) if self._split2 else self.z2
        self.xs2 = None if self._split2 else torch.empty(max(1, self.s2), self.o, **f32)
        self._lp1 = self._lp2 = None
        self._lp1_blocks = self._lp2_blocks = 0
        if self._fuse_l2:
            self._slot2, self._cnt_signed2 = _loss_slots(self.t2, self.idx2, self.s2, dev)
            if self._fuse_wg2:
                self._lp2_blocks = lib.gd_del_loss_bwd_wgrad_parts(self.s2, self.o)
                lp2_size = lib.gd_rows_gemm_wgrad_blocks(self.s2)
            else:
                self._lp2_blocks = lp2_size = lib.gd_del_loss_bwd_blocks(self.s2)
            self._lp2 = torch.zeros(2 * max(1, lp2_size + self.t2.outside_blocks()), **f32)
            self.dz2c = torch.zeros(self.s2, self.o, **f32)
        self.pre1 = torch.empty(n, self.h, **f32) if self._split1 else self.z1
        self._sel1 = m1.to(torch.uint8).contiguous() if self._split1 else None
        self.xs1 = None if self._split1 else torch.empty(max(1, self.s1), self.h, **f32)
        self.dz1 = torch.zeros(n, self.h, **f32)
        if isinstance(conv2, SAGEConv):
            self.dcat = torch.zeros(n, 2 * self.o, **f32)
            self.dz2 = self.dcat[:, self.o:]
        else:
            self.dz2 = torch.zeros(n, self.o, **f32)
        self.dh = torch.zeros(n, self.h, **f32)
        self.z1_pos = torch.zeros(max(1, self.s1), (self.h + 31) // 32, dtype=torch.int32, device=dev)
        self.g1 = torch.zeros_like(self.wd1)
        self.g2 = torch.zeros_like(self.wd2)
        self.sums = torch.zeros(4, **f32)
        self.ws1 = torch.empty(max(1, lib.gd_rows_gemm_wgrad_workspace(self.s1, self.h, self.h)), **f32)
        self.ws2 = torch.empty(max(1, lib.gd_rows_gemm_wgrad_workspace(self.s2, self.o, self.o)), **f32)
        self.iter_ctr = torch.zeros(1, dtype=torch.int32, device=dev)
        self.adam1, self.adam2 = _Adam(self.wd1, lr, iter_ctr=self.iter_ctr), _Adam(self.wd2, lr, iter_ctr=self.iter_ctr)
        self.hist = torch.zeros(history, 4, **f32)
        self.hist_pos = torch.zeros(1, dtype=torch.int32, device=dev)
        self.steps_done = 0
        self._graph = self._graph_k = None
        self._use_graph = use_graph
        self._const_refs = {}
        if self._fuse_loss1:
            self._slot1, self._cnt_signed1 = _loss_slots(self.t1, self.idx1, self.s1, dev)
            self._lp1_blocks = lib.gd_del1_loss_wgrad_parts(self.s1) if self._fuse_del1 else lib.gd_rows_gemm_wgrad_blocks(self.s1)
            self._lp1 = torch.zeros(2 * max(1, lib.gd_rows_gemm_wgrad_blocks(self.s1) + self.t1.outside_blocks()), **f32)
        self._tail_acc = [0, 0]
        self._arrive = torch.zeros(2, dtype=torch.int32, device=dev)
        self._gat_bufs = self._dt2_keep = None
        if self._chain1 and self._mode == 'gat':
            self._gat_bufs = {'dh': torch.zeros(n, self.o, **f32), 'da_src': torch.zeros(n, **f32), 'da_dst': torch.zeros(n, **f32)}
        elif self._chain1:
            self._dt2_keep = torch.zeros(n, self.o, **f32)
        self._fold2 = plan_del2_fold(self.facts, self.forms, lib.gd_del_loss_fold_wgrad_covers(self.s2, self.o, self.h), read_del2_fold())
        self._w2fold = torch.zeros(self.o, self.h, **f32) if self._fold2 else None
        self._gat_r1 = None
        if self._mode == 'gat':
            w2_ = conv2.lin_src.weight.detach()
            self._gat_r1 = ((conv2.att_src.detach().reshape(1, -1) @ w2_).reshape(-1).float().contiguous(),
                            (conv2.att_dst.detach().reshape(1, -1) @ w2_).reshape(-1).float().contiguous())
        if self._mode == 'rgcn':
            from .graph import TypedNodeCSR
            self.typed = TypedNodeCSR(edge_index, edge_type.to(dev), n, conv2.num_relations)
            self.typed_s1 = None
            if self._rgcn_rows_only and self.s1 > 0:
                in1 = torch.zeros(n, dtype=torch.bool, device=dev)
                in1[self.idx1.long()] = True
                self.typed_s1 = self.typed.restrict_bwd(in1)
            self._hbuf = torch.zeros(n, self.h, **f32)
            self._dxbuf = torch.zeros(n, self.h, **f32)
            for c_, din, dout, tr in ((conv1, self.x.shape[1], self.h, 0), (conv2, self.h, self.o, 0), (conv2, self.o, self.h, 1)):
                if int(lib.gd_rgcn_tile_kl(din, dout, c_.num_blocks or 1, tr)) > 0 and not knobs.rgcn_node_major:
                    tg_ = self.typed_s1 if (tr and self.typed_s1 is not None) else self.typed
                    if ops.rgcn_wave_form(din, dout, c_.num_blocks or 1, n, din) and self.typed.num_relations < 65536:
                        tg_.wave_plan(bool(tr))
                    else:
                        tg_.tile_plan(bool(tr))
                    ops.rgcn_packed_weight(c_.weight.detach(), c_.num_blocks or 1, din, dout, tr)
        if self._mode == 'sage':
            self._w2cat = torch.cat([conv2.lin_l.weight.detach(), conv2.lin_r.weight.detach()], 0).contiguous()
        if self._rows_only:
            from .graph import SplitPlan
            self._plan2 = SplitPlan(self.graph.rowptr, rows=self.idx2)
            self._plan_t1 = SplitPlan(self.graph.rowptr_t, rows=self.idx1)
            self._t1buf = torch.zeros(n, self.h, **f32)
            self._t1rbuf = torch.zeros(n, self.h, **f32) if self._mode == 'sage' else None
            self._t2buf = torch.zeros(n, self.o * (2 if self._mode == 'sage' else 1), **f32)
            self._dt2buf = self._dt2_keep if self._dt2_keep is not None else torch.zeros(n, self.o, **f32)
            self._adots = torch.zeros(2, n, **f32)
            if self._split1:
                self.pre1.zero_()
            self.p2.zero_()
        self.cache_layer1 = cache_layer1
        if cache_layer1:
            with torch.no_grad():
                self._conv1_forward()
                if self._split1:
                    self.p1 = self.pre1
                else:
                    self.p1 = self.z1.clone()
                    if self.s1:
                        self.xs1.copy_(self.p1[self.idx1.long()])

    def _affected_rows_closed(self):
        g, n, dev = self.graph, self.n, self.x.device
        in2 = torch.zeros(n, dtype=torch.bool, device=dev)
        in2[self.idx2.long()] = True
        in1_rows = torch.zeros(n, dtype=torch.bool, device=dev)
        in1_rows[self.idx1.long()] = True
        deg = (g.rowptr[1:] - g.rowptr[:-1]).long()
        erow = torch.repeat_interleave(torch.arange(n, device=dev), deg)
        closed = bool(in2[g.col.long()[in2[erow]]].all()) and bool(in2[self.idx1.long()].all())
        deg_t = (g.rowptr_t[1:] - g.rowptr_t[:-1]).long()
        erow_t = torch.repeat_interleave(torch.arange(n, device=dev), deg_t)
        return closed and bool(in2[g.col_t.long()[in1_rows[erow_t]]].all())

    @staticmethod
    def _mfma_weight(weight):
        out_f, in_f = weight.shape
        return in_f % 32 == 0 and out_f % 32 == 0 and out_f <= 128 and in_f * out_f * 4 <= 64 * 1024

    def _linear(self, x, weight, relu_in=False, idx=None, out=None):
        out_f, in_f = weight.shape
        if idx is not None or self._mfma_weight(weight):
            return ops.rows_gemm(x, idx, weight, trans_w=True, const_w=True, relu_in=relu_in, out=out)
        if ops.mfma_out_width(out_f):
            xin = torch.relu(x) if relu_in else x
            return ops.gemm_wide(xin, ops._const_weight(weight, True)[0], const_x=not relu_in, const_w=True)
        if in_f <= 1024:
            return ops.rows_gemm(x, None, weight, trans_w=True, const_w=True, relu_in=relu_in)
        raise NotImplementedError(f'NodeembEngine: a {in_f} -> {out_f} Linear has no kernel (inputs above 1,024 floats need an output '
                                  'width in {32, 64, 96, 128}); there is no vendor-BLAS fallback')

    def _linear_relu_z1(self, weight, idx=None, out=None):
        if not self._split1:
            return self._linear(self.z1, weight, relu_in=True, idx=idx, out=out)
        if idx is not None or self._mfma_weight(weight):
            return ops.rows_gemm_select(self.pre1, self.z1, self._sel1, weight, trans_w=True, const_w=True, relu_in=True,
                                        out=out, idx=idx)
        z = torch.where(self._sel1.bool()[:, None], self.z1, self.pre1)
        return self._linear(z, weight, relu_in=True)

    def _layer1_rows(self, weight):
        if self._rows_only and self._split1 and self._mfma_weight(weight):
            return self.idx2, self._t1buf, self._plan2
        return None, None, None

    def _conv1_forward(self):
        c = self.model.conv1
        g = self.graph
        if self._mode == 'rgcn':
            self._rgcn_conv(c, self.x, self.pre1, 0)
        elif self._mode == 'gcn':
            idx, out, plan = self._layer1_rows(c.lin.weight)
            self._spmm(False, g.val, self._linear(self.x, c.lin.weight, idx=idx, out=out), self.pre1, c.bias, 0.0, plan=plan)
        elif self._mode == 'gin':
            lin = c.nn
            if lin.out_features <= lin.in_features:
                idx, out, plan = self._layer1_rows(lin.weight)
                self._spmm(False, None, self._linear(self.x, lin.weight, idx=idx, out=out), self.pre1, lin.bias, 1.0 + c.eps, plan=plan)
            else:
                agg = torch.empty_like(self.x)
                self._spmm(False, None, self.x, agg, None, 1.0 + c.eps)
                ops.rows_gemm(agg, None, lin.weight, trans_w=True, const_w=True, bias=lin.bias, out=self.pre1)
        elif self._mode == 'sage':
            idx, out, plan = self._layer1_rows(c.lin_l.weight)
            t_l = self._linear(self.x, c.lin_l.weight, idx=idx, out=out)
            if (idx is None and self._mfma_weight(c.lin_r.weight)
                    and ops.rows_gemm_accumulate_ok(self.n, c.lin_r.weight.shape[1], c.lin_r.weight.shape[0])
                    and not self.knobs.sage_root_in_spmm):
                self._spmm(False, g.val, t_l, self.pre1, c.lin_l.bias, 0.0)
                ops.rows_gemm_accumulate_(self.pre1, self.x, None, c.lin_r.weight, trans_w=True, const_w=True)
            else:
                t_r = self._linear(self.x, c.lin_r.weight, idx=idx, out=None if idx is None else self._t1rbuf)
                self._spmm(False, g.val, t_l, self.pre1, c.lin_l.bias, 1.0, x_self=t_r, plan=plan)
        else:
            wsrc = c.lin_src.weight
            idx, out, _ = self._layer1_rows(wsrc)
            if idx is None and self._gat_dots and ops.rows_gemm_dots_ok(wsrc.shape[1], wsrc.shape[0], self.n):
                h1, a_src, a_dst = ops.rows_gemm_dots(self.x, wsrc, c.att_src, c.att_dst, const_w=True)
            else:
                h1 = self._linear(self.x, wsrc, idx=idx, out=out)
                a_src, a_dst = ops.row_dots(h1, c.att_src, c.att_dst)
            ops.gat_forward_raw(g, h1, a_src, a_dst, c.bias, c.negative_slope, out=self.pre1,
                                plan=self._plan2 if (self._rows_only and self._split1) else None)

    def _rgcn_conv(self, conv, inp, out, trans, relu_in=False):
        tg = self.typed
        nb = conv.num_blocks or 1
        ops.rows_gemm(inp, None, conv.root.detach(), trans_w=bool(trans), bias=None if trans else conv.bias.detach(), out=out,
                      relu_in=relu_in)
        ops.rgcn_typed_accumulate(tg, inp, conv.weight.detach(), nb, int(trans), out, relu_in=relu_in)

    def _conv2_forward(self):
        c = self.model.conv2
        if self._mode == 'rgcn':
            if self._split1:
                torch.where(self._sel1.bool()[:, None], self.z1, self.pre1, out=self._hbuf)
                self._hbuf.clamp_(min=0)
                self._rgcn_conv(c, self._hbuf, self.p2, 0)
            elif ops.rgcn_wave_relu_ok(self.typed, self.z1, self.p2, c.num_blocks or 1) and not self.knobs.rgcn_relu_pass:
                self._rgcn_conv(c, self.z1, self.p2, 0, relu_in=True)
            else:
                torch.clamp(self.z1, min=0, out=self._hbuf)
                self._rgcn_conv(c, self._hbuf, self.p2, 0)
        elif self._mode in ('gcn', 'gin', 'sage'):
            idx, out, plan = (self.idx2, self._t2buf, self._plan2) if self._rows_only else (None, None, None)
            if self._mode == 'gcn':
                self._spmm(False, self.graph.val, self._linear_relu_z1(c.lin.weight, idx, out), self.p2, c.bias, 0.0, plan=plan)
            elif self._mode == 'gin':
                lin = c.nn
                if lin.out_features > lin.in_features:
                    raise NotImplementedError('GIN layer that widens its input is not on the fused path')
                self._spmm(False, None, self._linear_relu_z1(lin.weight, idx, out), self.p2, lin.bias, 1.0 + c.eps, plan=plan)
            else:
                t2 = self._linear_relu_z1(self._w2cat, idx, out)
                self._spmm(False, self.graph.val, t2[:, :self.o], self.p2, c.lin_l.bias, 1.0, x_self=t2[:, self.o:], plan=plan)
        else:
            wsrc = c.lin_src.weight
            if self._gat_dots and self._split1 and ops.rows_gemm_dots_ok(wsrc.shape[1], wsrc.shape[0], self.s2 if self._rows_only else self.n,
                                                                        selected=self._rows_only):
                ro = self._rows_only
                h2, self._a_src, self._a_dst = ops.rows_gemm_dots(
                    self.pre1, wsrc, c.att_src, c.att_dst, inp_alt=self.z1, sel=self._sel1, relu_in=True, const_w=True,
                    out=self._t2buf if ro else None, idx=self.idx2 if ro else None,
                    dots_out=(self._adots[0], self._adots[1]) if ro else None)
            else:
                h2 = self._linear_relu_z1(wsrc)
                self._a_src, self._a_dst = ops.row_dots(h2, c.att_src, c.att_dst)
            self._h2 = h2
            _, self._rowmax, self._rowsum = ops.gat_forward_raw(self.graph, h2, self._a_src, self._a_dst, c.bias,
                                                                c.negative_slope, out=self.p2,
                                                                plan=self._plan2 if self._rows_only else None)

    def _conv2_backward_to_s1(self):
        c = self.model.conv2
        g = self.graph
        if self._mode == 'rgcn':
            if self.typed_s1 is not None:
                ops.rows_gemm(self.dz2, self.idx1, c.root.detach(), trans_w=True, out=self._dxbuf)
                ops.rgcn_typed_accumulate(self.typed_s1, self.dz2, c.weight.detach(), c.num_blocks or 1, 1, self._dxbuf)
            else:
                self._rgcn_conv(c, self.dz2, self._dxbuf, 1)
            ops.gate_rows(self._dxbuf, self.idx1, self.z1_pos, self.dh)
            return
        if self._mode == 'sage':
            self._spmm(True, g.val_t, self.dz2, self.dcat[:, :self.o], None, 0.0,
                       plan=self._plan_t1 if self._rows_only else None)
            dt2, w2 = self.dcat, self._w2cat
        elif self._mode in ('gcn', 'gin'):
            chain = self._chain1
            if self._rows_only:
                dt2, plan = self._dt2buf, self._plan_t1
            else:
                dt2, plan = (self._dt2_keep if chain else torch.empty(self.n, self.o, dtype=torch.float32, device=self.x.device)), None
            if self._mode == 'gcn':
                self._spmm(True, g.val_t, self.dz2, dt2, None, 0.0, plan=plan)
                w2 = c.lin.weight
            else:
                self._spmm(True, None, self.dz2, dt2, None, 1.0 + c.eps, plan=plan)
                w2 = c.nn.weight
            if chain:
                return
        else:
            chain = self._chain1
            dt2, da_s, da_d = ops.gat_backward_raw(g, self._h2, self._a_src, self._a_dst, self._rowmax, self._rowsum,
                                                   self.dz2, c.negative_slope,
                                                   plan=self._plan2 if self._rows_only else None,
                                                   plan_t=self._plan_t1 if self._rows_only else None,
                                                   bufs=self._gat_bufs if chain else None)
            if chain:
                return
            w2 = c.lin_src.weight
            if self._mfma_weight(w2) and not self.knobs.no_gat_rank1_epilogue:
                ops.rows_gemm(dt2, self.idx1, w2, trans_w=False, out=self.dh, gate_bits=self.z1_pos,
                              rank1=(da_s, self._gat_r1[0], da_d, self._gat_r1[1]))
                return
            ops.rank1_add2_(dt2, da_s, c.att_src, da_d, c.att_dst)
        ops.rows_gemm(dt2, self.idx1, w2, trans_w=False, out=self.dh, gate_bits=self.z1_pos)

    def _spmm(self, transposed, val, x, y, bias, self_coef, x_self=None, plan=None):
        g = self.graph
        if transposed:
            ops._spmm_raw(g.rowptr_t, g.col_t, val, x, bias, self_coef, self.n, plan or g.plan_t, out=y, x_self=x_self)
        else:
            ops._spmm_raw(g.rowptr, g.col, val, x, bias, self_coef, self.n, plan or g.plan, out=y, x_self=x_self)

    def _wgrad(self, a_compact, g, g_idx, n_sel, out, accumulate, ws, adam=None, g_add=None, a_idx=None):
        d_a, d_b = a_compact.shape[1], g.shape[1]
        if adam is not None:
            adam.applied += 1
        if adam is None or self._tail:
            if adam is not None:
                self._tail_acc[0 if adam is self.adam1 else 1] = int(accumulate)
            check(_lib.lib().gd_rows_gemm_wgrad_f32(ptr(a_compact), a_compact.stride(0), ptr(a_idx), ptr(g), g.stride(0),
                                                    ptr(g_idx), None, ptr(g_add), n_sel, d_a, d_b, ptr(out) if adam is None else None,
                                                    int(accumulate), ptr(ws), stream_ptr(g.device)),
                  'gd_rows_gemm_wgrad_f32')
            return
        check(_lib.lib().gd_rows_gemm_wgrad_adam_f32(
            ptr(a_compact), a_compact.stride(0), ptr(a_idx), ptr(g), g.stride(0), ptr(g_idx), None, ptr(g_add), n_sel,
            d_a, d_b, ptr(out), int(accumulate), ptr(ws), ptr(adam.param), ptr(adam.m), ptr(adam.v),
            ptr(adam.iter_ctr), adam.lr, adam.betas[0], adam.betas[1], adam.eps, stream_ptr(g.device)),
            'gd_rows_gemm_wgrad_adam_f32')

    def _wgrad1(self, accumulate, g_add):
        a1, a1_idx = (self.pre1, self.idx1) if self._split1 else (self.xs1, None)
        if not self._fuse_loss1:
            self._wgrad(a1, self.dz1, self.idx1, self.s1, self.g1, accumulate, self.ws1, adam=self.adam1,
                        g_add=g_add, a_idx=a1_idx)
            return
        a = self.adam1
        a.applied += 1
        if self._tail:
            self._tail_acc[0] = int(accumulate)
        check(_lib.lib().gd_rows_gemm_wgrad_loss_f32(
            ptr(a1), a1.stride(0), ptr(a1_idx), ptr(self.z1), self.z1.stride(0), ptr(self.idx1),
            ptr(self._slot1), ptr(self.t1.tm), ptr(self.t1.coef), ptr(self._cnt_signed1), ptr(g_add), self.s1, self.h,
            self.h, None if self._tail else ptr(self.g1), int(accumulate), ptr(self.ws1), ptr(self._lp1),
            None if self._tail else ptr(a.param), ptr(a.m), ptr(a.v),
            ptr(a.iter_ctr), a.lr, a.betas[0], a.betas[1], a.eps, stream_ptr(self.x.device)),
            'gd_rows_gemm_wgrad_loss_f32')

    def _iteration(self):
        lt = self.loss_type
        with torch.no_grad(), ops.keep_constants(self._const_refs):
            if not self.cache_layer1:
                self._conv1_forward()
            if self.cache_layer1 and not self._split1:
                ops.rows_gemm(self.p1, self.idx1, self.wd1, out=self.z1, sign_bits=self.z1_pos)
            elif self._fuse_del1:
                self._del1_fused(self.dh if lt == 'both_layerwise' else None)
            else:
                ops.rows_gemm(self.pre1, self.idx1, self.wd1, out=self.z1, save_in=self.xs1, sign_bits=self.z1_pos)
            fused_fin = self.t1.folded and self.t2.folded
            if not fused_fin:
                self.sums.zero_()
            s1 = None if fused_fin else self.sums[0:2]
            s2 = None if fused_fin else self.sums[2:4]
            if not self._fuse_loss1 and lt != 'only2_all':
                self.t1.launch(self.z1, self.dz1, s1)
            elif self._out1 and lt != 'only2_all' and not self._out_pair:
                self.t1.launch_outside(self.z1, None, self._lp1[2 * self._lp1_blocks:])
            if self._fuse_del1:
                pass
            elif lt == 'both_layerwise':
                self._wgrad1(False, self.dh)
            elif lt == 'only1':
                self._wgrad1(False, None)
            self._conv2_forward()
            if self._fuse_l2:
                self._del2_fused()
                if self._out2 and self._out_pair and lt != 'only2_all':
                    check(_lib.lib().gd_rowtarget_mse_pair_f32(
                        *self.t1.outside_args(self.z1, None, self._lp1[2 * self._lp1_blocks:]),
                        *self.t2.outside_args(self.p2, self.dz2, self._lp2[2 * self._lp2_blocks:]), stream_ptr(self.x.device)),
                        'gd_rowtarget_mse_pair_f32')
                elif self._out2:
                    self.t2.launch_outside(self.p2, self.dz2, self._lp2[2 * self._lp2_blocks:])
            else:
                ops.rows_gemm(self.p2, self.idx2, self.wd2, out=self.z2, save_in=self.xs2)
                self.t2.launch(self.z2, self.dz2, s2)
            if lt == 'both_layerwise':
                self._layer2_backward()
            elif lt == 'both_all':
                self._layer2_backward(g2_accumulate=True)
                self._wgrad1(True, self.dh)
            elif lt == 'only2_layerwise':
                self._layer2_backward(to_w1=False)
            elif lt == 'only2_all':
                self._layer2_backward()
                a1, a1_idx = (self.pre1, self.idx1) if self._split1 else (self.xs1, None)
                self._wgrad(a1, self.dh, self.idx1, self.s1, self.g1, False, self.ws1, adam=self.adam1, a_idx=a1_idx)
            if lt != 'only1' and not self._fuse_l2 and not self._tail:
                self.adam2.apply(self.g2)
            p1, n1 = ((self._lp1, self._lp1_blocks + (self.t1.outside_blocks() if self._out1 else 0)) if self._fuse_loss1
                      else (self.t1.partials, self.t1.n_partial_blocks()))
            p2, n2 = ((self._lp2, self._lp2_blocks + (self.t2.outside_blocks() if self._out2 else 0)) if self._fuse_l2
                      else (self.t2.partials, self.t2.n_partial_blocks()))
            if self._tail:
                a1, a2 = self.adam1, self.adam2
                lib_ = _lib.lib()
                nw1 = self._lp1_blocks if self._fuse_del1 else lib_.gd_rows_gemm_wgrad_blocks(self.s1)
                check(lib_.gd_step_tail_parts_f32(
                    ptr(self.ws1), nw1, self.h, self._tail_acc[0], ptr(self.g1), ptr(a1.param), ptr(a1.m), ptr(a1.v),
                    ptr(self.ws2), self._lp2_blocks if self._fuse_wg2 else lib_.gd_rows_gemm_wgrad_blocks(self.s2), self.o,
                    self._tail_acc[1], ptr(self.g2), ptr(a2.param),
                    ptr(a2.m), ptr(a2.v), a1.lr, a1.betas[0], a1.betas[1], a1.eps, ptr(p1), n1, ptr(p2), n2, ptr(self.hist),
                    self.hist.shape[0], ptr(self.hist_pos), ptr(self.iter_ctr), ptr(self._arrive), stream_ptr(self.x.device)),
                    'gd_step_tail_parts_f32')
            else:
                check(_lib.lib().gd_loss_finalize_f32(
                    ptr(p1) if fused_fin else None, n1 if fused_fin else 0,
                    ptr(p2) if fused_fin else None, n2 if fused_fin else 0,
                    None if fused_fin else ptr(self.sums), ptr(self.hist), self.hist.shape[0], ptr(self.hist_pos),
                    ptr(self.iter_ctr), stream_ptr(self.x.device)), 'gd_loss_finalize_f32')
            if self._user_wd2 is not None:
                self._user_wd2.data.copy_(self.wd2.data[:self._o_true, :self._o_true])

    def _conv2_weight(self):
        c2 = self.model.conv2
        return (c2.lin if self._mode == 'gcn' else c2.nn).weight.detach()

    def _del1_fused(self, g_add):
        self.adam1.applied += 1
        self._tail_acc[0] = 0
        if self._chain1:
            c2 = self.model.conv2
            if self._mode == 'gat':
                w_next, dt = c2.lin_src.weight.detach(), self._gat_bufs['dh']
                rank1 = (ptr(self._gat_bufs['da_src']), ptr(self._gat_r1[0]), ptr(self._gat_bufs['da_dst']), ptr(self._gat_r1[1]))
            else:
                w_next, dt = self._conv2_weight(), self._dt2_keep
                if self._fold2:
                    w_next = self._w2fold
                rank1 = (None, None, None, None)
            check(_lib.lib().gd_del1_chain_loss_wgrad_f32(
                ptr(self.pre1), self.pre1.stride(0), ptr(self.idx1), self.s1, ptr(self.wd1), self.h, ptr(self.z1), self.z1.stride(0),
                ptr(self.z1_pos), ptr(self._slot1), ptr(self.t1.tm), ptr(self.t1.coef), ptr(self._cnt_signed1), ptr(dt),
                dt.stride(0), self.o, ptr(w_next), *rank1, ptr(self._lp1), ptr(self.ws1), self._lp1_blocks,
                stream_ptr(self.x.device)), 'gd_del1_chain_loss_wgrad_f32')
            return
        check(_lib.lib().gd_del1_loss_wgrad_f32(
            ptr(self.pre1), self.pre1.stride(0), ptr(self.idx1), self.s1, ptr(self.wd1), self.h, ptr(self.z1), self.z1.stride(0),
            ptr(self.z1_pos), ptr(self._slot1), ptr(self.t1.tm), ptr(self.t1.coef), ptr(self._cnt_signed1), ptr(g_add),
            g_add.stride(0) if g_add is not None else 0, ptr(self._lp1), ptr(self.ws1), self._lp1_blocks, stream_ptr(self.x.device)),
            'gd_del1_loss_wgrad_f32')

    def _del2_fused(self):
        if self._fold2:
            w2 = self._conv2_weight()
            check(_lib.lib().gd_del_loss_fold_wgrad_parts_f32(
                ptr(self.p2), self.p2.stride(0), ptr(self.idx2), self.s2, ptr(self.wd2), self.o, ptr(self._slot2),
                ptr(self.t2.tm), ptr(self.t2.coef), ptr(self._cnt_signed2), ptr(self.dz2), self.dz2.stride(0), ptr(w2), self.h,
                ptr(self._w2fold), ptr(self._lp2), ptr(self.ws2), self._lp2_blocks, stream_ptr(self.x.device)),
                'gd_del_loss_fold_wgrad_parts_f32')
            return
        if self._fuse_wg2:
            check(_lib.lib().gd_del_loss_bwd_wgrad_parts_f32(
                ptr(self.p2), self.p2.stride(0), ptr(self.idx2), self.s2, ptr(self.wd2), self.o, ptr(self._slot2),
                ptr(self.t2.tm), ptr(self.t2.coef), ptr(self._cnt_signed2), None, self.o,
                ptr(self.dz2), self.dz2.stride(0), ptr(self._lp2), ptr(self.ws2), self._lp2_blocks, stream_ptr(self.x.device)),
                'gd_del_loss_bwd_wgrad_parts_f32')
            return
        check(_lib.lib().gd_del_loss_bwd_f32(
            ptr(self.p2), self.p2.stride(0), ptr(self.idx2), self.s2, ptr(self.wd2), self.o, ptr(self._slot2),
            ptr(self.t2.tm), ptr(self.t2.coef), ptr(self._cnt_signed2), ptr(self.dz2c), self.dz2c.stride(0),
            ptr(self.dz2), self.dz2.stride(0), ptr(self._lp2), stream_ptr(self.x.device)), 'gd_del_loss_bwd_f32')

    def _layer2_backward(self, to_w1=True, g2_accumulate=False):
        if self._fuse_wg2:
            self.adam2.applied += 1
            self._tail_acc[1] = int(g2_accumulate)
        elif self._fuse_l2:
            self._wgrad(self.p2, self.dz2c, None, self.s2, self.g2, g2_accumulate, self.ws2, a_idx=self.idx2,
                        adam=self.adam2)
        elif self._split2:
            self._wgrad(self.p2, self.dz2, self.idx2, self.s2, self.g2, g2_accumulate, self.ws2, a_idx=self.idx2,
                        adam=self.adam2 if self._tail else None)
        else:
            self._wgrad(self.xs2, self.dz2, self.idx2, self.s2, self.g2, g2_accumulate, self.ws2,
                        adam=self.adam2 if self._tail else None)
        if not to_w1:
            return
        if not self._fuse_l2:
            ops.rows_gemm(self.dz2, self.idx2, self.wd2, trans_w=True, out=self.dz2)
        self._conv2_backward_to_s1()

    def step(self):
        if not self._use_graph:
            self._iteration()
        elif self._graph is None:
            self._capture()
            self._graph.replay()
        else:
            self._graph.replay()
        self.steps_done += 1

    def run(self, n_steps, unroll=4):
        if not self._use_graph or unroll <= 1:
            for _ in range(n_steps):
                self.step()
            return
        if n_steps >= unroll:
            self.prepare_unrolled(unroll)
            while n_steps >= unroll:
                self._graph_k[1].replay()
                self.steps_done += unroll
                n_steps -= unroll
        for _ in range(n_steps):
            self.step()

    def prepare_unrolled(self, unroll):
        if not self._use_graph or unroll <= 1:
            return
        if self._graph is None:
            self._capture()
        if self._graph_k is None or self._graph_k[0] != unroll:
            self._graph_k = (unroll, capture_iterations(self._iteration, self._mutable_state, unroll, warm_up=False))

    def _mutable_state(self):
        state = [self.wd1.data, self.wd2.data, self.g1, self.g2, self.adam1.m, self.adam1.v, self.iter_ctr,
                 self.adam2.m, self.adam2.v, self.hist, self.hist_pos, self.dz1, self.dz2, self.dh]
        if self._chain1:
            state += [self.z1_pos] + ([self._dt2_keep] if self._dt2_keep is not None else
                                      [self._gat_bufs[k] for k in ('dh', 'da_src', 'da_dst')])
        if self._fold2:
            state.append(self._w2fold)
        state.append(self._arrive)
        if self._user_wd2 is not None:
            state.append(self._user_wd2.data)
        return state

    def _capture(self):
        self._graph = capture_iterations(self._iteration, self._mutable_state)

    def loss_history(self):
        k = min(self.steps_done, self.hist.shape[0])
        s = self.hist[:k].double().cpu()
        nan = float('nan')
        fam = self.family
        r1 = logged_loss(fam, s[:, 0], self.t1.k_const[0], self.t1.n_r) if self.t1.count_r else s[:, 0] * nan
        l1 = logged_loss(fam, s[:, 1], self.t1.k_const[1], self.t1.n_l) if self.t1.count_l else s[:, 1] * nan
        r2 = logged_loss(fam, s[:, 2], self.t2.k_const[0], self.t2.n_r) if self.t2.count_r else s[:, 2] * nan
        l2 = logged_loss(fam, s[:, 3], self.t2.k_const[1], self.t2.n_l) if self.t2.count_l else s[:, 3] * nan
        a, lt = self.alpha, self.loss_type
        if lt in ('both_all', 'both_layerwise'):
            loss_r, loss_l = r1 + r2, l1 + l2
            loss = a * loss_r + (1 - a) * loss_l
        elif lt == 'only2_layerwise':
            loss_r, loss_l = r1 + r2, l1 + l2
            loss = a * r2 + (1 - a) * l2
        elif lt == 'only2_all':
            loss_r, loss_l = r2, l2
            loss = l2 + a * r2
        else:
            loss_r, loss_l = r1, l1
            loss = l1 + a * r1
        return torch.stack([loss, loss_r, loss_l], 1)
```

### include/gnndelete_hip.h

```cpp
#ifndef GNNDELETE_HIP_H
#define GNNDELETE_HIP_H

#include <stdint.h>

#ifdef __cplusplus
extern "C" {
#endif

#define GD_ABI_VERSION 9

enum {
  GD_OK = 0,
  GD_E_NULL = 1,
  GD_E_DIM = 2,
  GD_E_ALIGN = 3,
  GD_E_WORKSPACE = 4
};

int gd_abi_version(void);
const char* gd_last_error_string(void);
const char* gd_build_source_hash(void);

#define GD_MATRIX_SPLIT_DEFAULT 0
int gd_matrix_split(void);
// ... 142 lines not shown
                           const float* w, int32_t d_in, int32_t d_out, int32_t trans_w,
                           const uint32_t* gate_bits, float* out, int64_t ld_out, void* stream);

int gd_gate_rows_f32(const float* src, int64_t ld_src, const int32_t* idx, int32_t n_sel, const uint32_t* gate_bits,
                     int32_t d, float* out, int64_t ld_out, void* stream);

int gd_rows_gemm_gated_rank1_f32(const float* in, int64_t ld_in, const int32_t* idx, int32_t n_sel,
                                 const float* w, int32_t d_in, int32_t d_out, int32_t trans_w,
                                 const uint32_t* gate_bits, const float* row_a, const float* col_p,
                                 const float* row_b, const float* col_q, float* out, int64_t ld_out, void* stream);

int64_t gd_rows_gemm_wgrad_workspace(int32_t n_sel, int32_t d_a, int32_t d_b);
int gd_rows_gemm_wgrad_f32(const float* a, int64_t ld_a, const int32_t* a_idx,
                           const float* g, int64_t ld_g, const int32_t* g_idx,
                           const float* relu_mask, const float* g_add, int32_t n_sel, int32_t d_a,
                           int32_t d_b, float* dw, int32_t accumulate, float* partials, void* stream);

int gd_rows_gemm_wgrad_adam_f32(const float* a, int64_t ld_a, const int32_t* a_idx,
                                const float* g, int64_t ld_g, const int32_t* g_idx,
                                const float* relu_mask, const float* g_add, int32_t n_sel, int32_t d_a,
                                int32_t d_b, float* dw, int32_t accumulate, float* partials,
                                float* param, float* exp_avg, float* exp_avg_sq, const int32_t* iter,
                                double lr, double beta1, double beta2, double eps, void* stream);

int gd_rows_gemm_wgrad_reduce_f32(const float* partials, int32_t n_sel, int32_t d_a, int32_t d_b, float* dw,
                                  int32_t accumulate, float* param, float* exp_avg, float* exp_avg_sq,
                                  const int32_t* iter, double lr, double beta1, double beta2, double eps, void* stream);

int gd_step_tail_f32(const float* partials1, int32_t n_sel1, int32_t d1, int32_t accumulate1, float* dw1, float* param1,
                     float* exp_avg1, float* exp_avg_sq1, const float* partials2, int32_t n_sel2, int32_t d2,
                     int32_t accumulate2, float* dw2, float* param2, float* exp_avg2, float* exp_avg_sq2, double lr,
                     double beta1, double beta2, double eps, const float* loss_partials1, int32_t n1,
                     const float* loss_partials2, int32_t n2, float* hist, int32_t capacity, int32_t* pos, int32_t* iter,
                     int32_t* arrive, void* stream);
int gd_step_tail_parts_f32(const float* partials1, int32_t n_part1, int32_t d1, int32_t accumulate1, float* dw1, float* param1,
                           float* exp_avg1, float* exp_avg_sq1, const float* partials2, int32_t n_part2, int32_t d2,
                           int32_t accumulate2, float* dw2, float* param2, float* exp_avg2, float* exp_avg_sq2, double lr,
                           double beta1, double beta2, double eps, const float* loss_partials1, int32_t n1,
                           const float* loss_partials2, int32_t n2, float* hist, int32_t capacity, int32_t* pos, int32_t* iter,
                           int32_t* arrive, void* stream);

int32_t gd_rows_gemm_wgrad_blocks(int32_t n_sel);
int gd_rows_gemm_wgrad_loss_f32(const float* a, int64_t ld_a, const int32_t* a_idx,
                                const float* z, int64_t ld_z, const int32_t* z_idx,
                                const int32_t* loss_slot, const float* tm, const float* coef,
                                const float* cnt_signed, const float* g_add,
                                int32_t n_sel, int32_t d_a, int32_t d_b, float* dw, int32_t accumulate,
                                float* partials, float* loss_partials,
                                float* param, float* exp_avg, float* exp_avg_sq, const int32_t* iter,
                                double lr, double beta1, double beta2, double eps, void* stream);

int32_t gd_del_loss_bwd_blocks(int32_t n_sel);
int gd_del_loss_bwd_f32(const float* p, int64_t ld_p, const int32_t* idx, int32_t n_sel, const float* w, int32_t d,
                        const int32_t* loss_slot, const float* tm, const float* coef, const float* cnt_signed,
                        float* dz, int64_t ld_dz, float* dp, int64_t ld_dp, float* loss_partials, void* stream);

int gd_del_loss_bwd_wgrad_f32(const float* p, int64_t ld_p, const int32_t* idx, int32_t n_sel, const float* w, int32_t d,
                              const int32_t* loss_slot, const float* tm, const float* coef, const float* cnt_signed,
                              float* dz, int64_t ld_dz, float* dp, int64_t ld_dp, float* loss_partials,
                              float* wgrad_partials, void* stream);
int32_t gd_del_loss_bwd_wgrad_parts(int32_t n_sel, int32_t d);
int gd_del_loss_bwd_wgrad_parts_f32(const float* p, int64_t ld_p, const int32_t* idx, int32_t n_sel, const float* w, int32_t d,
                                    const int32_t* loss_slot, const float* tm, const float* coef, const float* cnt_signed,
                                    float* dz, int64_t ld_dz, float* dp, int64_t ld_dp, float* loss_partials,
                                    float* wgrad_partials, int32_t n_part, void* stream);
int32_t gd_del_loss_fold_wgrad_covers(int32_t n_sel, int32_t d, int32_t h);
int gd_del_loss_fold_wgrad_parts_f32(const float* p, int64_t ld_p, const int32_t* idx, int32_t n_sel, const float* w, int32_t d,
                                     const int32_t* loss_slot, const float* tm, const float* coef, const float* cnt_signed,
                                     float* g, int64_t ld_g, const float* w_next, int32_t h, float* w_fold,
                                     float* loss_partials, float* wgrad_partials, int32_t n_part, void* stream);

int32_t gd_del1_loss_wgrad_covers(int32_t n_sel, int32_t d);
int32_t gd_del1_loss_wgrad_parts(int32_t n_sel);
int gd_del1_loss_wgrad_f32(const float* p, int64_t ld_p, const int32_t* idx, int32_t n_sel, const float* w, int32_t d, float* z,
                           int64_t ld_z, uint32_t* sign_out, const int32_t* loss_slot, const float* tm, const float* coef,
                           const float* cnt_signed, const float* g_add, int64_t ld_gadd, float* loss_partials,
                           float* wgrad_partials, int32_t n_part, void* stream);
int gd_del1_chain_loss_wgrad_f32(const float* p, int64_t ld_p, const int32_t* idx, int32_t n_sel, const float* w, int32_t d, float* z,
                                 int64_t ld_z, uint32_t* sign_io, const int32_t* loss_slot, const float* tm, const float* coef,
                                 const float* cnt_signed, const float* dt, int64_t ld_dt, int32_t d_next, const float* w_next,
                                 const float* row_a, const float* col_a, const float* row_b, const float* col_b,
                                 float* loss_partials, float* wgrad_partials, int32_t n_part, void* stream);


int64_t gd_rowpair_mse_workspace(int32_t n_seg);
int gd_rowpair_mse_f32(const float* z, int64_t ld_z, const float* o, int64_t ld_o, int32_t d,
                       const int32_t* seg_ptr, const int32_t* seg_row, int32_t n_seg,
                       const int32_t* term_o, const float* term_w, const int32_t* term_kind,
                       float* dz, int64_t ld_dz, int32_t dz_compact,
                       float* sums, float* partials, void* stream);

int64_t gd_rowtarget_mse_workspace(int32_t n_rows);
int gd_rowtarget_mse_f32(const float* z, int64_t ld_z, const float* tm, int32_t d,
                         const int32_t* row_idx, const float* coef, const float* cnt, const int32_t* kind,
                         int32_t n_rows, float* dz, int64_t ld_dz, float* sums, float* partials, void* stream);
int32_t gd_rowtarget_mse_pair_covers(int32_t d_a, int32_t d_b);
int gd_rowtarget_mse_pair_f32(const float* z_a, int64_t ld_z_a, const float* tm_a, int32_t d_a, const int32_t* row_idx_a,
                              const float* coef_a, const float* cnt_a, const int32_t* kind_a, int32_t n_rows_a, float* dz_a,
                              int64_t ld_dz_a, float* partials_a, const float* z_b, int64_t ld_z_b, const float* tm_b, int32_t d_b,
                              const int32_t* row_idx_b, const float* coef_b, const float* cnt_b, const int32_t* kind_b,
                              int32_t n_rows_b, float* dz_b, int64_t ld_dz_b, float* partials_b, void* stream);

int32_t gd_rowtarget_mse_blocks(int32_t n_rows);
int gd_loss_finalize_f32(const float* partials1, int32_t n1, const float* partials2, int32_t n2,
                         const float* extra_sums, float* hist, int32_t capacity, int32_t* pos, int32_t* iter,
                         void* stream);

int32_t gd_rowfold_loss_blocks(int32_t n_rows);
int gd_rowfold_loss_f32(int32_t family, const float* z, int64_t ld_z, const float* tm, int32_t d, int32_t d_valid,
                        const int32_t* row_idx, const float* coef, const float* cnt, const int32_t* kind, int32_t n_rows,
                        float* dz, int64_t ld_dz, float* partials, void* stream);
int gd_rowfold_kld_scale_f32(const float* partials, int32_t n_blocks, float k_dec, float k_ni, float inv_n_dec, float inv_n_ni,
                             const int32_t* row_idx, const int32_t* kind, int32_t n_rows, int32_t d, float* dz, int64_t ld_dz,
                             float* scales, void* stream);

int64_t gd_gemm_f32_workspace(int32_t n_rows, int32_t k, int32_t n);
int gd_gemm_f32(const float* in, int64_t ld_in, const int32_t* idx, int32_t n_rows, const float* w, int32_t k,
                int32_t n, const float* bias, float* out, int64_t ld_out, float* workspace, void* stream);

int gd_edge_dot_f32(const float* z, int64_t ld_z, int32_t d, const int64_t* e0, const int64_t* e1,
                    const float* rel, int64_t ld_rel, const int64_t* etype,
                    int64_t n_edges, float* out, void* stream);

int gd_edge_dot_bwd_f32(const float* z, int64_t ld_z, int32_t d, const int32_t* other, const float* w,
                        const float* rel, int64_t ld_rel, const int32_t* etype, const int64_t* inc_ptr,
                        int64_t n_nodes, float* dz, int64_t ld_dz, void* stream);

int64_t gd_pairs_sigmoid_mse_workspace(int32_t n_s, int32_t d);
int gd_pairs_sigmoid_mse_f32(const float* z, int64_t ld_z, const int32_t* nodes, int32_t n_s, int32_t d,
                             const float* target, int64_t ld_t, float inv_count,
                             float* loss, float* dz, float* workspace, void* stream);


int64_t gd_edgeprob_dec_workspace(int64_t m, int32_t d);
int gd_edgeprob_dec_f32(const float* z, int64_t ld_z, int64_t n_nodes, int32_t d, const int64_t* pos, int64_t ld_pos,
                        const int64_t* neg, int64_t ld_neg, int64_t m, float coef, float* w, float* loss,
                        const int32_t* src_edge, const int64_t* inc_ptr, float* w_inc, float* workspace, void* stream);

int64_t gd_edge_incidence_workspace(int64_t n_nodes, int64_t n_edges);
int gd_edge_incidence(const int64_t* e0, const int64_t* e1, int64_t n_edges, int64_t n_nodes, int64_t* inc_ptr,
                      int32_t* other, int32_t* src_edge, void* workspace, int64_t workspace_bytes, void* stream);

int64_t gd_edge_incidence_fixed_bytes(int64_t n_nodes, int64_t n_fixed);
int gd_edge_incidence_fixed(const int64_t* e0, const int64_t* e1, int64_t n_fixed, int64_t n_nodes, void* image, int64_t image_bytes,
                            void* workspace, int64_t workspace_bytes, void* stream);
int64_t gd_edge_incidence_update_workspace(int64_t n_nodes, int64_t n_edges);
int gd_edge_incidence_update(const void* image, const int64_t* e0, const int64_t* e1, int64_t n_fixed, int64_t n_edges,
                             int64_t n_nodes, int64_t* inc_ptr, int32_t* other, int32_t* src_edge, void* workspace,
                             int64_t workspace_bytes, void* stream);

int gd_rows_add_f32(float* dz, int64_t ld_dz, int64_t n_rows, const int32_t* nodes, int32_t n_s, const float* src,
                    int64_t ld_src, float scale, int32_t d, void* stream);

int gd_edgeprob_record_f32(const float* loss_r, const float* loss_l, float coef_r, float coef_l, float* hist,
                           int32_t capacity, int32_t* pos, void* stream);

int64_t gd_edgeprob_batch_loss_workspace(int64_t k, int64_t n_cand, int32_t d);
int gd_edgeprob_batch_loss_f32(const float* z, int64_t ld_z, int64_t n_nodes, const float* z_ori, int64_t ld_ori, int64_t n_ori,
                               int32_t d, const int64_t* pos, int64_t ld_pos, const int64_t* neg, int64_t ld_neg, int64_t k,
                               const int64_t* cand_src, const int64_t* cand_dst, int64_t n_cand, float coef_e, float coef_l,
                               int64_t* dec, int64_t ld_dec, float* w, float* losses, int64_t* inc_ptr, int32_t* other,
                               int32_t* src_edge, float* w_inc, void* inc_workspace, int64_t inc_workspace_bytes,
                               float* workspace, void* stream);


int64_t gd_edge_bce_workspace(int64_t m_all, int32_t d);
// ... 67 lines not shown
```

Measured before the change: 1938 iters/s.

## Fold layer-1 linear and deletion operator into one weight for Del-1 chain

Precomputes a folded weight and bias combining the frozen layer-1 linear with the trainable deletion weight, so the chained Del-1 pass works directly on the aggregated features A·X instead of first forming pre1 on the deleted rows. The kernel gains a FOLD variant that seeds the MFMA accumulators with the folded bias, accumulates column sums for the bias gradient, and writes transposed weight-gradient partials. A new step-tail kernel reduces these partials, applies Adam, and refreshes the folded weight and bias each step. Layer-1 pre-activation is then only computed for the complementary rows. The cost is extra LDS, more tail-kernel work and more complex bookkeeping.

```diff
diff --git a/gnndelete_amd/_lib.py b/gnndelete_amd/_lib.py
--- a/gnndelete_amd/_lib.py
+++ b/gnndelete_amd/_lib.py
@@ -101,6 +101,12 @@
     'gd_del1_loss_wgrad_covers': (ctypes.c_int32, [_i32, _i32]),
     'gd_del1_loss_wgrad_parts': (ctypes.c_int32, [_i32]),
     'gd_del1_chain_loss_wgrad_f32': (ctypes.c_int, [_p, _i64, _p, _i32, _p, _i32, _p, _i64, _p, _p, _p, _p, _p, _p, _i64, _i32, _p, _p, _p, _p, _p, _p, _p, _i32, _p]),
+    'gd_del1_chain_fold_covers': (ctypes.c_int32, [_i32, _i32, _i32]),
+    'gd_del1_chain_fold_loss_wgrad_f32': (ctypes.c_int, [_p, _i64, _p, _i32, _p, _p, _i32, _p, _i64, _p, _p, _p, _p, _p, _p, _i64, _i32, _p, _p,
+                                                         _p, _p, _i32, _p]),
+    'gd_layer1_fold_f32': (ctypes.c_int, [_p, _p, _p, _p, _p, _p]),
+    'gd_step_tail_fold1_f32': (ctypes.c_int, [_p, _p, _i32, _i32, _i32, _p, _p, _p, _p, _p, _p, _p, _p, _p, _i32, _i32, _i32, _p, _p, _p, _p,
+                                              _f64, _f64, _f64, _f64, _p, _i32, _p, _i32, _p, _i32, _p, _p, _p, _p]),
     'gd_del1_loss_wgrad_f32': (ctypes.c_int, [_p, _i64, _p, _i32, _p, _i32, _p, _i64, _p, _p, _p, _p, _p, _p, _i64, _p, _p, _i32, _p]),
     'gd_rowtarget_mse_blocks': (_i32, [_i32]),
     'gd_rowfold_loss_blocks': (_i32, [_i32]),
diff --git a/gnndelete_amd/csrc/del_fused.hip b/gnndelete_amd/csrc/del_fused.hip
--- a/gnndelete_amd/csrc/del_fused.hip
+++ b/gnndelete_amd/csrc/del_fused.hip
@@ -603,12 +603,14 @@
 }
 
 struct ChainRank1 { const float* ra; const float* ua; const float* rb; const float* ub; };
-template <bool RANK1>
+struct ChainFold { const float* bias; float* colsum; };
+template <bool RANK1, bool FOLD = false>
 __global__ __launch_bounds__(256) __attribute__((amdgpu_waves_per_eu(1, 1))) void del1_chain_ws_kernel(
     const float* __restrict__ p, int64_t ld_p, const int32_t* __restrict__ idx, int32_t n_sel, const float* __restrict__ w,
     float* __restrict__ z, int64_t ld_z, uint32_t* __restrict__ sign_io, DelLoss loss, const float* __restrict__ dt, int64_t ld_dt,
-    const float* __restrict__ w_next, float* __restrict__ wg_partials, int32_t n_part, ChainRank1 r1) {
+    const float* __restrict__ w_next, float* __restrict__ wg_partials, int32_t n_part, ChainRank1 r1, ChainFold fo) {
   constexpr int D = 128, H = 64, PTP = 144, PTZ = 80;
+  constexpr int RT = D + 4;
   constexpr int kTiles = 4 * (16 * PTP + 16 * PTZ);
   extern __shared__ __attribute__((aligned(16))) float wl[];
   __shared__ float lred[2][4];
@@ -660,6 +662,16 @@
   float4 x[8], dv[4], tv[4];
   float4 ua4[RANK1 ? 4 : 1], ub4[RANK1 ? 4 : 1];
   float ra_row = 0.f, rb_row = 0.f;
+  f32x4w bias4[FOLD ? 4 : 1];
+  float csum[FOLD ? 4 : 1];
+  if (FOLD) {
+#pragma unroll
+    for (int t = 0; t < 4; ++t) {
+      const float4 b4 = *reinterpret_cast<const float4*>(fo.bias + cb + 16 * t + 4 * kq);
+      bias4[t] = f32x4w{b4.x, b4.y, b4.z, b4.w};
+      csum[t] = 0.f;
+    }
+  }
   if (RANK1) {
 #pragma unroll
     for (int t = 0; t < 4; ++t) {
@@ -719,7 +731,7 @@
             for (int t = 0; t < 4; ++t) {
               const float4 wf = wq[i & 1][t];
               const float wa = c == 0 ? wf.x : c == 1 ? wf.y : c == 2 ? wf.z : wf.w;
-              if (i == 0 && c == 0) acc[t] = __builtin_amdgcn_mfma_f32_16x16x4f32(wa, xv[0], f32x4w{0.f, 0.f, 0.f, 0.f}, 0, 0, 0);
+              if (i == 0 && c == 0) acc[t] = __builtin_amdgcn_mfma_f32_16x16x4f32(wa, xv[0], FOLD ? bias4[FOLD ? t : 0] : f32x4w{0.f, 0.f, 0.f, 0.f}, 0, 0, 0);
               else acc[t] = __builtin_amdgcn_mfma_f32_16x16x4f32(wa, xv[c], acc[t], 0, 0, 0);
             }
         }
@@ -766,8 +778,9 @@
           dq.x = fmaf(rb_c, ub4[t].x, fmaf(ra_c, ua4[t].x, dq.x)); dq.y = fmaf(rb_c, ub4[t].y, fmaf(ra_c, ua4[t].y, dq.y));
           dq.z = fmaf(rb_c, ub4[t].z, fmaf(ra_c, ua4[t].z, dq.z)); dq.w = fmaf(rb_c, ub4[t].w, fmaf(ra_c, ua4[t].w, dq.w));
         }
-        const float4 gv = make_float4(cf * d4.x + ((m & 1u) ? dq.x : 0.f), cf * d4.y + ((m & 2u) ? dq.y : 0.f),
-                                      cf * d4.z + ((m & 4u) ? dq.z : 0.f), cf * d4.w + ((m & 8u) ? dq.w : 0.f));
+        float4 gv = make_float4(cf * d4.x + ((m & 1u) ? dq.x : 0.f), cf * d4.y + ((m & 2u) ? dq.y : 0.f),
+                                cf * d4.z + ((m & 4u) ? dq.z : 0.f), cf * d4.w + ((m & 8u) ? dq.w : 0.f));
+        if (FOLD) gv = make_float4(livef * gv.x, livef * gv.y, livef * gv.z, livef * gv.w);
         *reinterpret_cast<float4*>(tz + r * PTZ + 16 * t + 4 * kq) = gv;
       }
       sq *= livef;
@@ -790,6 +803,10 @@
         for (int ta = 0; ta < 8; ++ta) a_op[ta] = tp[(4 * sp + kq) * PTP + 16 * ta + r];
 #pragma unroll
         for (int tb = 0; tb < 4; ++tb) b_op[tb] = tz[(4 * sp + kq) * PTZ + 16 * tb + r];
+        if (FOLD) {
+#pragma unroll
+          for (int tb = 0; tb < 4; ++tb) csum[tb] += b_op[tb];
+        }
 #pragma unroll
         for (int ta = 0; ta < 8; ++ta)
 #pragma unroll
@@ -803,19 +820,46 @@
   }
   __syncthreads();
   float* const red = wl;
-#pragma unroll
-  for (int ta = 0; ta < 8; ++ta)
-#pragma unroll
-    for (int tb = 0; tb < 4; ++tb)
-#pragma unroll
-      for (int v = 0; v < 4; ++v) red[wave * D * H + (16 * ta + 4 * kq + v) * H + 16 * tb + r] = gacc[ta * 4 + tb][v];
-  __syncthreads();
-  for (int slot = blockIdx.x; slot < n_part; slot += gridDim.x) {
-    float* const out = wg_partials + (int64_t)slot * D * D;
-    const bool mine = slot == (int)blockIdx.x;
-    for (int e = tid; e < D * D; e += 256) {
-      const int i = e >> 7, c = e & 127, hf = c >> 6, ch = c & 63;
-      out[e] = mine ? red[hf * D * H + i * H + ch] + red[(2 + hf) * D * H + i * H + ch] : 0.f;
+  if (FOLD) {
+    float* const cred = wl + 4 * H * RT;
+#pragma unroll
+    for (int ta = 0; ta < 8; ++ta)
+#pragma unroll
+      for (int tb = 0; tb < 4; ++tb)
+        *reinterpret_cast<float4*>(red + wave * H * RT + (16 * tb + r) * RT + 16 * ta + 4 * kq) =
+            make_float4(gacc[ta * 4 + tb][0], gacc[ta * 4 + tb][1], gacc[ta * 4 + tb][2], gacc[ta * 4 + tb][3]);
+#pragma unroll
+    for (int tb = 0; tb < 4; ++tb) {
+      float cs = csum[FOLD ? tb : 0];
+      cs += __shfl_xor(cs, 16);
+      cs += __shfl_xor(cs, 32);
+      if (kq == 0) cred[wave * H + 16 * tb + r] = cs;
+    }
+    __syncthreads();
+    for (int slot = blockIdx.x; slot < n_part; slot += gridDim.x) {
+      float* const out = wg_partials + (int64_t)slot * D * D;
+      const bool mine = slot == (int)blockIdx.x;
+      for (int e = tid; e < D * D; e += 256) {
+        const int c = e >> 7, i = e & 127, hf = c >> 6, ch = c & 63;
+        out[e] = mine ? red[hf * H * RT + ch * RT + i] + red[(2 + hf) * H * RT + ch * RT + i] : 0.f;
+      }
+      if (tid < D) fo.colsum[(int64_t)slot * D + tid] = mine ? cred[(tid >> 6) * H + (tid & 63)] + cred[(2 + (tid >> 6)) * H + (tid & 63)] : 0.f;
+    }
+  } else {
+#pragma unroll
+    for (int ta = 0; ta < 8; ++ta)
+#pragma unroll
+      for (int tb = 0; tb < 4; ++tb)
+#pragma unroll
+        for (int v = 0; v < 4; ++v) red[wave * D * H + (16 * ta + 4 * kq + v) * H + 16 * tb + r] = gacc[ta * 4 + tb][v];
+    __syncthreads();
+    for (int slot = blockIdx.x; slot < n_part; slot += gridDim.x) {
+      float* const out = wg_partials + (int64_t)slot * D * D;
+      const bool mine = slot == (int)blockIdx.x;
+      for (int e = tid; e < D * D; e += 256) {
+        const int i = e >> 7, c = e & 127, hf = c >> 6, ch = c & 63;
+        out[e] = mine ? red[hf * D * H + i * H + ch] + red[(2 + hf) * D * H + i * H + ch] : 0.f;
+      }
     }
   }
   ls0 = wave_sum(ls0);
@@ -1050,12 +1094,43 @@
     static const hipError_t at = hipFuncSetAttribute(reinterpret_cast<const void*>(&del1_chain_ws_kernel<true>), hipFuncAttributeMaxDynamicSharedMemorySize, kLds);
     if (at != hipSuccess) return fail(-(int)at, "%s: %s", name, hipGetErrorString(at));
     hipLaunchKernelGGL(del1_chain_ws_kernel<true>, dim3(grid), dim3(256), kLds, (hipStream_t)stream, p, ld_p, idx, n_sel, w, z, ld_z, sign_io, loss, dt,
-                       ld_dt, w_next, wgrad_partials, n_part, r1);
+                       ld_dt, w_next, wgrad_partials, n_part, r1, ChainFold{nullptr, nullptr});
   } else {
     static const hipError_t at = hipFuncSetAttribute(reinterpret_cast<const void*>(&del1_chain_ws_kernel<false>), hipFuncAttributeMaxDynamicSharedMemorySize, kLds);
     if (at != hipSuccess) return fail(-(int)at, "%s: %s", name, hipGetErrorString(at));
     hipLaunchKernelGGL(del1_chain_ws_kernel<false>, dim3(grid), dim3(256), kLds, (hipStream_t)stream, p, ld_p, idx, n_sel, w, z, ld_z, sign_io, loss, dt,
-                       ld_dt, w_next, wgrad_partials, n_part, r1);
+                       ld_dt, w_next, wgrad_partials, n_part, r1, ChainFold{nullptr, nullptr});
   }
   return launched("del1_chain_ws");
 }
+
+extern "C" int32_t gd_del1_chain_fold_covers(int32_t n_sel, int32_t d, int32_t h) {
+  return gd_del1_loss_wgrad_covers(n_sel, h) && d == 128 ? 1 : 0;
+}
+
+extern "C" int gd_del1_chain_fold_loss_wgrad_f32(const float* a, int64_t ld_a, const int32_t* idx, int32_t n_sel, const float* w_fold,
+                                                 const float* bias_fold, int32_t d, float* z, int64_t ld_z, uint32_t* sign_io,
+                                                 const int32_t* loss_slot, const float* tm, const float* coef, const float* cnt_signed,
+                                                 const float* dt, int64_t ld_dt, int32_t d_next, const float* w_next, float* loss_partials,
+                                                 float* wgrad_partials_t, float* colsum_partials, int32_t n_part, void* stream) {
+  using namespace gd;
+  const char* name = "gd_del1_chain_fold_loss_wgrad_f32";
+  if (n_sel == 0) return GD_OK;
+  GD_REQUIRE(a && idx && w_fold && bias_fold && z && sign_io && loss_slot && tm && coef && cnt_signed && dt && w_next && loss_partials &&
+                 wgrad_partials_t && colsum_partials, GD_E_NULL, "%s: null pointer", name);
+  GD_REQUIRE(d == 128 && d_next == 64, GD_E_DIM, "%s: widths %d / %d must be 128 / 64", name, d, d_next);
+  GD_REQUIRE(ld_a >= d && ld_z >= d && ld_dt >= d_next && ld_a % 4 == 0 && ld_z % 4 == 0 && ld_dt % 4 == 0, GD_E_DIM, "%s: bad row strides", name);
+  GD_REQUIRE(aligned16(a) && aligned16(z) && aligned16(tm) && aligned16(dt) && aligned16(wgrad_partials_t) && aligned16(bias_fold) &&
+                 (reinterpret_cast<uintptr_t>(sign_io) & 7u) == 0, GD_E_ALIGN, "%s: unaligned", name);
+  GD_REQUIRE(a != z && dt != z, GD_E_DIM, "%s: z must not alias a or dt", name);
+  GD_REQUIRE(n_part >= 1 && n_part <= gd_rows_gemm_wgrad_blocks(n_sel), GD_E_DIM,
+             "%s: n_part=%d outside [1, gd_rows_gemm_wgrad_blocks(n_sel)=%d]", name, n_part, gd_rows_gemm_wgrad_blocks(n_sel));
+  const DelLoss loss{loss_slot, tm, coef, cnt_signed, loss_partials};
+  const int grid = ws_cu_count() < n_part ? ws_cu_count() : n_part;
+  constexpr int kLds = (4 * (16 * 144 + 16 * 80) + 128 * 128 + 64 * 128) * 4;
+  static const hipError_t at = hipFuncSetAttribute(reinterpret_cast<const void*>(&del1_chain_ws_kernel<false, true>), hipFuncAttributeMaxDynamicSharedMemorySize, kLds);
+  if (at != hipSuccess) return fail(-(int)at, "%s: %s", name, hipGetErrorString(at));
+  hipLaunchKernelGGL((del1_chain_ws_kernel<false, true>), dim3(grid), dim3(256), kLds, (hipStream_t)stream, a, ld_a, idx, n_sel, w_fold, z, ld_z, sign_io, loss,
+                     dt, ld_dt, w_next, wgrad_partials_t, n_part, ChainRank1{nullptr, nullptr, nullptr, nullptr}, ChainFold{bias_fold, colsum_partials});
+  return launched("del1_chain_fold_ws");
+}
diff --git a/gnndelete_amd/csrc/rows_gemm.hip b/gnndelete_amd/csrc/rows_gemm.hip
--- a/gnndelete_amd/csrc/rows_gemm.hip
+++ b/gnndelete_amd/csrc/rows_gemm.hip
@@ -673,58 +673,54 @@
   float* hist; int32_t capacity; int32_t* pos; int32_t* iter; int32_t* arrive;
 };
 
-__global__ __launch_bounds__(256) void step_tail_kernel(TailJob j1, TailJob j2, TailFin fin, double lr, double beta1, double beta2,
-                                                        double eps) {
-  __shared__ float4 red[16][16];
-  __shared__ float fred[4][256];
-  __shared__ int32_t t_sh;
-  const int nb1 = (j1.n_elem / 4 + 15) / 16, nb2 = (j2.n_elem / 4 + 15) / 16;
+__device__ __forceinline__ int32_t tail_check_in(const TailFin& fin) {
+  int32_t t = atomicAdd(fin.iter, 0);
+  asm volatile("" : "+v"(t));
+  atomicAdd(fin.arrive + (t < 0 ? 1 : 0), 1);
+  return t + 1;
+}
+
+__device__ __forceinline__ void tail_job_block(const TailJob& j, int blk, const TailFin& fin, float4 (*red)[16], int32_t* t_sh, double lr,
+                                               double beta1, double beta2, double eps) {
   const int tid = threadIdx.x;
-  if ((int)blockIdx.x < nb1 + nb2) {
-    const bool first = (int)blockIdx.x < nb1;
-    const TailJob j = first ? j1 : j2;
-    const int blk = first ? blockIdx.x : blockIdx.x - nb1;
-    if (tid == 0) {
-      int32_t t = atomicAdd(fin.iter, 0);
-      asm volatile("" : "+v"(t));
-      atomicAdd(fin.arrive + (t < 0 ? 1 : 0), 1);
-      t_sh = t + 1;
-    }
-    const int vv = tid & 15, slice = tid >> 4;
-    const int e4 = blk * 16 + vv;
-    const int n4 = j.n_elem >> 2;
-    float4 s0 = f4_zero(), s1 = f4_zero(), s2 = f4_zero(), s3 = f4_zero();
-    if (e4 < n4) {
-      int b = slice;
-      for (; b + 48 < j.n_part; b += 64) {
-        const float4 p0 = reinterpret_cast<const float4*>(j.partials + (int64_t)b * j.n_elem)[e4];
-        const float4 p1 = reinterpret_cast<const float4*>(j.partials + (int64_t)(b + 16) * j.n_elem)[e4];
-        const float4 p2 = reinterpret_cast<const float4*>(j.partials + (int64_t)(b + 32) * j.n_elem)[e4];
-        const float4 p3 = reinterpret_cast<const float4*>(j.partials + (int64_t)(b + 48) * j.n_elem)[e4];
-        s0 = f4_add(s0, p0); s1 = f4_add(s1, p1); s2 = f4_add(s2, p2); s3 = f4_add(s3, p3);
-      }
-      for (; b < j.n_part; b += 16) s0 = f4_add(s0, reinterpret_cast<const float4*>(j.partials + (int64_t)b * j.n_elem)[e4]);
-    }
-    red[slice][vv] = f4_add(f4_add(s0, s1), f4_add(s2, s3));
-    __syncthreads();
-    if (slice == 0 && e4 < n4) {
-      float4 t4 = j.accumulate ? reinterpret_cast<float4*>(j.dw)[e4] : f4_zero();
-#pragma unroll
-      for (int i = 0; i < 16; ++i) t4 = f4_add(t4, red[i][vv]);
-      reinterpret_cast<float4*>(j.dw)[e4] = t4;
-      const AdamScalars sc = adam_scalars(lr, beta1, beta2, eps, t_sh);
-      float4 p4 = reinterpret_cast<float4*>(j.param)[e4], m4 = reinterpret_cast<float4*>(j.m)[e4],
-             v4 = reinterpret_cast<float4*>(j.v)[e4];
-      adam_update(p4.x, m4.x, v4.x, t4.x, sc);
-      adam_update(p4.y, m4.y, v4.y, t4.y, sc);
-      adam_update(p4.z, m4.z, v4.z, t4.z, sc);
-      adam_update(p4.w, m4.w, v4.w, t4.w, sc);
-      reinterpret_cast<float4*>(j.param)[e4] = p4;
-      reinterpret_cast<float4*>(j.m)[e4] = m4;
-      reinterpret_cast<float4*>(j.v)[e4] = v4;
-    }
-    return;
-  }
+  if (tid == 0) *t_sh = tail_check_in(fin);
+  const int vv = tid & 15, slice = tid >> 4;
+  const int e4 = blk * 16 + vv;
+  const int n4 = j.n_elem >> 2;
+  float4 s0 = f4_zero(), s1 = f4_zero(), s2 = f4_zero(), s3 = f4_zero();
+  if (e4 < n4) {
+    int b = slice;
+    for (; b + 48 < j.n_part; b += 64) {
+      const float4 p0 = reinterpret_cast<const float4*>(j.partials + (int64_t)b * j.n_elem)[e4];
+      const float4 p1 = reinterpret_cast<const float4*>(j.partials + (int64_t)(b + 16) * j.n_elem)[e4];
+      const float4 p2 = reinterpret_cast<const float4*>(j.partials + (int64_t)(b + 32) * j.n_elem)[e4];
+      const float4 p3 = reinterpret_cast<const float4*>(j.partials + (int64_t)(b + 48) * j.n_elem)[e4];
+      s0 = f4_add(s0, p0); s1 = f4_add(s1, p1); s2 = f4_add(s2, p2); s3 = f4_add(s3, p3);
+    }
+    for (; b < j.n_part; b += 16) s0 = f4_add(s0, reinterpret_cast<const float4*>(j.partials + (int64_t)b * j.n_elem)[e4]);
+  }
+  red[slice][vv] = f4_add(f4_add(s0, s1), f4_add(s2, s3));
+  __syncthreads();
+  if (slice == 0 && e4 < n4) {
+    float4 t4 = j.accumulate ? reinterpret_cast<float4*>(j.dw)[e4] : f4_zero();
+#pragma unroll
+    for (int i = 0; i < 16; ++i) t4 = f4_add(t4, red[i][vv]);
+    reinterpret_cast<float4*>(j.dw)[e4] = t4;
+    const AdamScalars sc = adam_scalars(lr, beta1, beta2, eps, *t_sh);
+    float4 p4 = reinterpret_cast<float4*>(j.param)[e4], m4 = reinterpret_cast<float4*>(j.m)[e4],
+           v4 = reinterpret_cast<float4*>(j.v)[e4];
+    adam_update(p4.x, m4.x, v4.x, t4.x, sc);
+    adam_update(p4.y, m4.y, v4.y, t4.y, sc);
+    adam_update(p4.z, m4.z, v4.z, t4.z, sc);
+    adam_update(p4.w, m4.w, v4.w, t4.w, sc);
+    reinterpret_cast<float4*>(j.param)[e4] = p4;
+    reinterpret_cast<float4*>(j.m)[e4] = m4;
+    reinterpret_cast<float4*>(j.v)[e4] = v4;
+  }
+}
+
+__device__ __forceinline__ void tail_finalize_block(const TailFin& fin, float (*fred)[256], int n_wait) {
+  const int tid = threadIdx.x;
   float a = 0.f, b = 0.f, c = 0.f, d = 0.f;
   for (int i = tid; i < fin.n1; i += 256) { a += fin.p1[2 * i]; b += fin.p1[2 * i + 1]; }
   for (int i = tid; i < fin.n2; i += 256) { c += fin.p2[2 * i]; d += fin.p2[2 * i + 1]; }
@@ -740,11 +736,146 @@
   if (tid < 4) fin.hist[(int64_t)(*fin.pos) * 4 + tid] = fred[tid][0];
   __syncthreads();
   if (tid == 0) {
-    while (atomicAdd(fin.arrive, 0) < nb1 + nb2) __builtin_amdgcn_s_sleep(8);
+    while (atomicAdd(fin.arrive, 0) < n_wait) __builtin_amdgcn_s_sleep(8);
     *fin.arrive = 0;
     *fin.pos = (*fin.pos + 1) % fin.capacity;
     atomicAdd(fin.iter, 1);
   }
+}
+
+__global__ __launch_bounds__(256) void step_tail_kernel(TailJob j1, TailJob j2, TailFin fin, double lr, double beta1, double beta2,
+                                                        double eps) {
+  __shared__ float4 red[16][16];
+  __shared__ float fred[4][256];
+  __shared__ int32_t t_sh;
+  const int nb1 = (j1.n_elem / 4 + 15) / 16, nb2 = (j2.n_elem / 4 + 15) / 16;
+  if ((int)blockIdx.x < nb1 + nb2) {
+    const bool first = (int)blockIdx.x < nb1;
+    tail_job_block(first ? j1 : j2, first ? blockIdx.x : blockIdx.x - nb1, fin, red, &t_sh, lr, beta1, beta2, eps);
+    return;
+  }
+  tail_finalize_block(fin, fred, nb1 + nb2);
+}
+
+__device__ __forceinline__ void fold1_column(const float* w1s, const float* __restrict__ b1, const float* wd_col, int c, float* scr,
+                                             float* __restrict__ wf, float* __restrict__ bf) {
+  const int tid = threadIdx.x, i = tid & 127, hf = tid >> 7;
+  float acc = 0.f;
+#pragma unroll 16
+  for (int j = 64 * hf; j < 64 * hf + 64; ++j) acc = fmaf(w1s[j * 129 + i], wd_col[j], acc);
+  scr[tid] = acc;
+  __syncthreads();
+  if (tid < 128) wf[(int64_t)tid * 128 + c] = scr[tid] + scr[tid + 128];
+  __syncthreads();
+  scr[tid] = tid < 128 ? b1[tid] * wd_col[tid] : 0.f;
+  __syncthreads();
+  for (int off = 64; off > 0; off >>= 1) {
+    if (tid < off) scr[tid] += scr[tid + off];
+    __syncthreads();
+  }
+  if (tid == 0) bf[c] = scr[0];
+  __syncthreads();
+}
+
+__device__ __forceinline__ void fold1_fetch_w1(const float* __restrict__ w1, float4 (&r)[16]) {
+#pragma unroll
+  for (int it = 0; it < 16; ++it) r[it] = reinterpret_cast<const float4*>(w1)[threadIdx.x + 256 * it];
+}
+__device__ __forceinline__ void fold1_store_w1(const float4 (&r)[16], float* w1s) {
+#pragma unroll
+  for (int it = 0; it < 16; ++it) {
+    const int e = threadIdx.x + 256 * it;
+    float* dst = w1s + (e >> 5) * 129 + (e & 31) * 4;
+    dst[0] = r[it].x; dst[1] = r[it].y; dst[2] = r[it].z; dst[3] = r[it].w;
+  }
+}
+
+__global__ __launch_bounds__(256) void layer1_fold_kernel(const float* __restrict__ w1, const float* __restrict__ b1, const float* __restrict__ wd,
+                                                          float* __restrict__ wf, float* __restrict__ bf) {
+  extern __shared__ __attribute__((aligned(16))) float w1s[];
+  __shared__ float wd_col[128];
+  __shared__ float scr[256];
+  const int c = blockIdx.x;
+  float4 w1r[16];
+  fold1_fetch_w1(w1, w1r);
+  if (threadIdx.x < 128) wd_col[threadIdx.x] = wd[(int64_t)threadIdx.x * 128 + c];
+  fold1_store_w1(w1r, w1s);
+  __syncthreads();
+  fold1_column(w1s, b1, wd_col, c, scr, wf, bf);
+}
+
+struct TailFold1 { const float* colsum; const float* w1; const float* b1; float* wf; float* bf; };
+
+__global__ __launch_bounds__(256) void step_tail_fold1_kernel(TailJob j1, TailJob j2, TailFin fin, TailFold1 fo, double lr, double beta1,
+                                                              double beta2, double eps) {
+  extern __shared__ __attribute__((aligned(16))) float w1s[];
+  __shared__ float4 red[16][16];
+  __shared__ float fred[4][256];
+  __shared__ float gcol[128], wd_col[128];
+  __shared__ int32_t t_sh;
+  constexpr int D = 128;
+  const int nb2 = (j2.n_elem / 4 + 15) / 16;
+  const int tid = threadIdx.x;
+  if ((int)blockIdx.x >= D + nb2) { tail_finalize_block(fin, fred, D + nb2); return; }
+  if ((int)blockIdx.x >= D) { tail_job_block(j2, blockIdx.x - D, fin, red, &t_sh, lr, beta1, beta2, eps); return; }
+  const int c = blockIdx.x;
+  if (tid == 0) t_sh = tail_check_in(fin);
+  float4 w1r[16];
+  fold1_fetch_w1(fo.w1, w1r);
+  {
+    const int vv = tid & 31, slice = tid >> 5;
+    const float4* src = reinterpret_cast<const float4*>(j1.partials + (int64_t)c * D) + vv;
+    const int64_t pitch4 = (int64_t)D * D / 4;
+    float4 sa[8];
+#pragma unroll
+    for (int q = 0; q < 8; ++q) sa[q] = f4_zero();
+    int b = slice;
+    for (; b + 56 < j1.n_part; b += 64) {
+      float4 pv[8];
+#pragma unroll
+      for (int q = 0; q < 8; ++q) pv[q] = src[(b + 8 * q) * pitch4];
+#pragma unroll
+      for (int q = 0; q < 8; ++q) sa[q] = f4_add(sa[q], pv[q]);
+    }
+    for (; b < j1.n_part; b += 8) sa[0] = f4_add(sa[0], src[b * pitch4]);
+    float4* const red8 = &red[0][0];
+    red8[slice * 32 + vv] = f4_add(f4_add(f4_add(sa[0], sa[1]), f4_add(sa[2], sa[3])), f4_add(f4_add(sa[4], sa[5]), f4_add(sa[6], sa[7])));
+    float cs = 0.f;
+    for (int q = tid; q < j1.n_part; q += 256) cs += fo.colsum[(int64_t)q * D + c];
+    fred[0][tid] = cs;
+    fold1_store_w1(w1r, w1s);
+    __syncthreads();
+    if (tid < 32) {
+      float4 t4 = red8[tid];
+#pragma unroll
+      for (int i = 1; i < 8; ++i) t4 = f4_add(t4, red8[i * 32 + tid]);
+      reinterpret_cast<float4*>(gcol)[tid] = t4;
+    }
+    for (int off = 128; off > 0; off >>= 1) {
+      if (tid < off) fred[0][tid] += fred[0][tid + off];
+      __syncthreads();
+    }
+  }
+  {
+    const int j = tid & 127, hf = tid >> 7;
+    float acc = 0.f;
+#pragma unroll 16
+    for (int i = 64 * hf; i < 64 * hf + 64; ++i) acc = fmaf(w1s[j * 129 + i], gcol[i], acc);
+    fred[1][tid] = acc;
+    __syncthreads();
+    if (tid < D) {
+      const float g = fmaf(fo.b1[tid], fred[0][0], fred[1][tid] + fred[1][tid + 128]);
+      const int64_t e = (int64_t)tid * D + c;
+      j1.dw[e] = g;
+      const AdamScalars sc = adam_scalars(lr, beta1, beta2, eps, t_sh);
+      float pv = j1.param[e], mv = j1.m[e], vv = j1.v[e];
+      adam_update(pv, mv, vv, g, sc);
+      j1.param[e] = pv; j1.m[e] = mv; j1.v[e] = vv;
+      wd_col[tid] = pv;
+    }
+    __syncthreads();
+  }
+  fold1_column(w1s, fo.b1, wd_col, c, fred[2], fo.wf, fo.bf);
 }
 
 __global__ __launch_bounds__(256) void wgrad_reduce_scalar_kernel(const float* __restrict__ partials, int32_t n_part,
@@ -1110,6 +1241,45 @@
                         hist, capacity, pos, iter, arrive, stream);
 }
 
+static constexpr int kFold1Lds = 128 * 129 * 4;
+
+extern "C" int gd_layer1_fold_f32(const float* w1, const float* b1, const float* wd, float* wf, float* bf, void* stream) {
+  using namespace gd;
+  GD_REQUIRE(w1 && b1 && wd && wf && bf, GD_E_NULL, "gd_layer1_fold_f32: null pointer");
+  static const hipError_t at = hipFuncSetAttribute(reinterpret_cast<const void*>(&layer1_fold_kernel), hipFuncAttributeMaxDynamicSharedMemorySize, kFold1Lds);
+  if (at != hipSuccess) return fail(-(int)at, "gd_layer1_fold_f32: %s", hipGetErrorString(at));
+  hipLaunchKernelGGL(layer1_fold_kernel, dim3(128), dim3(256), kFold1Lds, (hipStream_t)stream, w1, b1, wd, wf, bf);
+  return launched("layer1_fold");
+}
+
+extern "C" int gd_step_tail_fold1_f32(const float* partials1_t, const float* colsum1, int32_t n_part1, int32_t d1, int32_t accumulate1,
+                                      const float* w1, const float* b1, float* dw1, float* param1, float* exp_avg1, float* exp_avg_sq1,
+                                      float* wf, float* bf, const float* partials2, int32_t n_part2, int32_t d2, int32_t accumulate2,
+                                      float* dw2, float* param2, float* exp_avg2, float* exp_avg_sq2, double lr, double beta1, double beta2,
+                                      double eps, const float* loss_partials1, int32_t n1, const float* loss_partials2, int32_t n2,
+                                      float* hist, int32_t capacity, int32_t* pos, int32_t* iter, int32_t* arrive, void* stream) {
+  using namespace gd;
+  const char* name = "gd_step_tail_fold1_f32";
+  GD_REQUIRE(partials1_t && colsum1 && w1 && b1 && wf && bf && dw1 && param1 && exp_avg1 && exp_avg_sq1 && partials2 && dw2 && param2 &&
+                 exp_avg2 && exp_avg_sq2, GD_E_NULL, "%s: null weight-gradient / optimizer pointer", name);
+  GD_REQUIRE(hist && pos && iter && arrive && capacity > 0 && (n1 == 0 || loss_partials1) && (n2 == 0 || loss_partials2), GD_E_NULL,
+             "%s: null bookkeeping pointer", name);
+  GD_REQUIRE(d1 == 128 && accumulate1 == 0, GD_E_DIM, "%s: the folded layer-1 job is 128 wide and does not accumulate (d1=%d accumulate1=%d)", name,
+             d1, accumulate1);
+  GD_REQUIRE(n_part1 > 0 && n_part2 > 0 && d2 > 0 && (d2 * d2) % 4 == 0, GD_E_DIM, "%s: bad part counts / widths", name);
+  GD_REQUIRE(aligned16(partials1_t) && aligned16(partials2) && aligned16(dw2), GD_E_ALIGN, "%s: unaligned", name);
+  const TailJob j1{partials1_t, n_part1, d1 * d1, 0, dw1, param1, exp_avg1, exp_avg_sq1};
+  const TailJob j2{partials2, n_part2, d2 * d2, accumulate2, dw2, param2, exp_avg2, exp_avg_sq2};
+  const TailFin fin{loss_partials1, n1, loss_partials2, n2, hist, capacity, pos, iter, arrive};
+  const TailFold1 fo{colsum1, w1, b1, wf, bf};
+  const int grid = 128 + (j2.n_elem / 4 + 15) / 16 + 1;
+  GD_REQUIRE(grid <= 1024, GD_E_DIM, "%s: Del weights too large for the co-resident grid (%d blocks)", name, grid);
+  static const hipError_t at = hipFuncSetAttribute(reinterpret_cast<const void*>(&step_tail_fold1_kernel), hipFuncAttributeMaxDynamicSharedMemorySize, kFold1Lds);
+  if (at != hipSuccess) return fail(-(int)at, "%s: %s", name, hipGetErrorString(at));
+  hipLaunchKernelGGL(step_tail_fold1_kernel, dim3(grid), dim3(256), kFold1Lds, (hipStream_t)stream, j1, j2, fin, fo, lr, beta1, beta2, eps);
+  return launched("step_tail_fold1");
+}
+
 extern "C" int32_t gd_rows_gemm_wgrad_blocks(int32_t n_sel) {
   int nb, rpb;
   gd::wgrad_geometry(n_sel, &nb, &rpb);
diff --git a/gnndelete_amd/engine.py b/gnndelete_amd/engine.py
--- a/gnndelete_amd/engine.py
+++ b/gnndelete_amd/engine.py
@@ -123,6 +123,16 @@
 
 def plan_del2_fold(facts, forms, covers, enabled=True):
     return bool(enabled and covers and forms.chain1 and facts.mode in ('gcn', 'gin') and forms.fuse_wg2 and not forms.out2)
+
+
+def read_layer1_fold(env=None):
+    env = os.environ if env is None else env
+    return env.get('GD_LAYER1_FOLD') != '0'
+
+
+def plan_layer1_fold(facts, forms, covers, enabled=True):
+    return bool(enabled and covers and forms.chain1 and forms.fuse_del1 and forms.split1 and facts.mode == 'gcn'
+                and facts.loss_type == 'both_layerwise' and not facts.cache_layer1 and facts.h == 128)
 
 
 def _loss_coefficients(loss_type, alpha):
@@ -557,6 +567,28 @@
             self._dt2_keep = torch.zeros(n, self.o, **f32)
         self._fold2 = plan_del2_fold(self.facts, self.forms, lib.gd_del_loss_fold_wgrad_covers(self.s2, self.o, self.h), read_del2_fold())
         self._w2fold = torch.zeros(self.o, self.h, **f32) if self._fold2 else None
+        self._fold1 = False
+        if self._mode == 'gcn':
+            w1_ = conv1.lin.weight
+            self._fold1 = plan_layer1_fold(
+                self.facts, self.forms,
+                tuple(w1_.shape) == (128, 128) and x.shape[1] == 128 and x.dtype == torch.float32
+                and bool(lib.gd_del1_chain_fold_covers(self.s1, x.shape[1], self.h)), read_layer1_fold())
+        if self._fold1:
+            self._w1 = conv1.lin.weight.detach().float().contiguous()
+            self._b1 = (conv1.bias.detach().float().contiguous() if conv1.bias is not None else torch.zeros(self.h, **f32))
+            self._a1 = torch.zeros(n, self.h, **f32)
+            self._wf, self._bf = torch.empty(self.h, self.h, **f32), torch.empty(self.h, **f32)
+            check(lib.gd_layer1_fold_f32(ptr(self._w1), ptr(self._b1), ptr(self.wd1), ptr(self._wf), ptr(self._bf), stream_ptr(dev)),
+                  'gd_layer1_fold_f32')
+            self._cs1 = torch.zeros(max(1, lib.gd_rows_gemm_wgrad_blocks(self.s1)) * self.h, **f32)
+            rest = torch.ones(n, dtype=torch.bool, device=dev)
+            if self._rows_only:
+                rest.zero_()
+                rest[self.idx2.long()] = True
+            rest[self.idx1.long()] = False
+            self._idx1c = rest.nonzero().flatten().to(torch.int32)
+            self.pre1.zero_()
         self._gat_r1 = None
         if self._mode == 'gat':
             w2_ = conv2.lin_src.weight.detach()
@@ -654,6 +686,10 @@
         g = self.graph
         if self._mode == 'rgcn':
             self._rgcn_conv(c, self.x, self.pre1, 0)
+        elif self._mode == 'gcn' and self._fold1:
+            self._spmm(False, g.val, self.x, self._a1, None, 0.0, plan=self._plan2 if self._rows_only else None)
+            if self._idx1c.numel():
+                ops.rows_gemm(self._a1, self._idx1c, self._w1, trans_w=True, const_w=True, bias=self._b1, out=self.pre1)
         elif self._mode == 'gcn':
             idx, out, plan = self._layer1_rows(c.lin.weight)
             self._spmm(False, g.val, self._linear(self.x, c.lin.weight, idx=idx, out=out), self.pre1, c.bias, 0.0, plan=plan)
@@ -808,6 +844,7 @@
             'gd_rows_gemm_wgrad_adam_f32')
 
     def _wgrad1(self, accumulate, g_add):
+        assert not self._fold1, 'the folded layer-1 step never forms pre1 on the Del-1 rows: its weight gradient comes out of the chained pass'
         a1, a1_idx = (self.pre1, self.idx1) if self._split1 else (self.xs1, None)
         if not self._fuse_loss1:
             self._wgrad(a1, self.dz1, self.idx1, self.s1, self.g1, accumulate, self.ws1, adam=self.adam1,
@@ -835,6 +872,7 @@
             elif self._fuse_del1:
                 self._del1_fused(self.dh if lt == 'both_layerwise' else None)
             else:
+                assert not self._fold1
                 ops.rows_gemm(self.pre1, self.idx1, self.wd1, out=self.z1, save_in=self.xs1, sign_bits=self.z1_pos)
             fused_fin = self.t1.folded and self.t2.folded
             if not fused_fin:
@@ -885,13 +923,22 @@
                 a1, a2 = self.adam1, self.adam2
                 lib_ = _lib.lib()
                 nw1 = self._lp1_blocks if self._fuse_del1 else lib_.gd_rows_gemm_wgrad_blocks(self.s1)
-                check(lib_.gd_step_tail_parts_f32(
-                    ptr(self.ws1), nw1, self.h, self._tail_acc[0], ptr(self.g1), ptr(a1.param), ptr(a1.m), ptr(a1.v),
-                    ptr(self.ws2), self._lp2_blocks if self._fuse_wg2 else lib_.gd_rows_gemm_wgrad_blocks(self.s2), self.o,
-                    self._tail_acc[1], ptr(self.g2), ptr(a2.param),
-                    ptr(a2.m), ptr(a2.v), a1.lr, a1.betas[0], a1.betas[1], a1.eps, ptr(p1), n1, ptr(p2), n2, ptr(self.hist),
-                    self.hist.shape[0], ptr(self.hist_pos), ptr(self.iter_ctr), ptr(self._arrive), stream_ptr(self.x.device)),
-                    'gd_step_tail_parts_f32')
+                if self._fold1:
+                    check(lib_.gd_step_tail_fold1_f32(
+                        ptr(self.ws1), ptr(self._cs1), nw1, self.h, self._tail_acc[0], ptr(self._w1), ptr(self._b1), ptr(self.g1),
+                        ptr(a1.param), ptr(a1.m), ptr(a1.v), ptr(self._wf), ptr(self._bf),
+                        ptr(self.ws2), self._lp2_blocks if self._fuse_wg2 else lib_.gd_rows_gemm_wgrad_blocks(self.s2), self.o,
+                        self._tail_acc[1], ptr(self.g2), ptr(a2.param), ptr(a2.m), ptr(a2.v), a1.lr, a1.betas[0], a1.betas[1], a1.eps,
+                        ptr(p1), n1, ptr(p2), n2, ptr(self.hist), self.hist.shape[0], ptr(self.hist_pos), ptr(self.iter_ctr),
+                        ptr(self._arrive), stream_ptr(self.x.device)), 'gd_step_tail_fold1_f32')
+                else:
+                    check(lib_.gd_step_tail_parts_f32(
+                        ptr(self.ws1), nw1, self.h, self._tail_acc[0], ptr(self.g1), ptr(a1.param), ptr(a1.m), ptr(a1.v),
+                        ptr(self.ws2), self._lp2_blocks if self._fuse_wg2 else lib_.gd_rows_gemm_wgrad_blocks(self.s2), self.o,
+                        self._tail_acc[1], ptr(self.g2), ptr(a2.param),
+                        ptr(a2.m), ptr(a2.v), a1.lr, a1.betas[0], a1.betas[1], a1.eps, ptr(p1), n1, ptr(p2), n2, ptr(self.hist),
+                        self.hist.shape[0], ptr(self.hist_pos), ptr(self.iter_ctr), ptr(self._arrive), stream_ptr(self.x.device)),
+                        'gd_step_tail_parts_f32')
             else:
                 check(_lib.lib().gd_loss_finalize_f32(
                     ptr(p1) if fused_fin else None, n1 if fused_fin else 0,
@@ -918,6 +965,13 @@
                 if self._fold2:
                     w_next = self._w2fold
                 rank1 = (None, None, None, None)
+            if self._fold1:
+                check(_lib.lib().gd_del1_chain_fold_loss_wgrad_f32(
+                    ptr(self._a1), self._a1.stride(0), ptr(self.idx1), self.s1, ptr(self._wf), ptr(self._bf), self.h, ptr(self.z1),
+                    self.z1.stride(0), ptr(self.z1_pos), ptr(self._slot1), ptr(self.t1.tm), ptr(self.t1.coef), ptr(self._cnt_signed1),
+                    ptr(dt), dt.stride(0), self.o, ptr(w_next), ptr(self._lp1), ptr(self.ws1), ptr(self._cs1), self._lp1_blocks,
+                    stream_ptr(self.x.device)), 'gd_del1_chain_fold_loss_wgrad_f32')
+                return
             check(_lib.lib().gd_del1_chain_loss_wgrad_f32(
                 ptr(self.pre1), self.pre1.stride(0), ptr(self.idx1), self.s1, ptr(self.wd1), self.h, ptr(self.z1), self.z1.stride(0),
                 ptr(self.z1_pos), ptr(self._slot1), ptr(self.t1.tm), ptr(self.t1.coef), ptr(self._cnt_signed1), ptr(dt),
@@ -1010,6 +1064,8 @@
                                       [self._gat_bufs[k] for k in ('dh', 'da_src', 'da_dst')])
         if self._fold2:
             state.append(self._w2fold)
+        if self._fold1:
+            state += [self._wf, self._bf]
         state.append(self._arrive)
         if self._user_wd2 is not None:
             state.append(self._user_wd2.data)
diff --git a/include/gnndelete_hip.h b/include/gnndelete_hip.h
--- a/include/gnndelete_hip.h
+++ b/include/gnndelete_hip.h
@@ -248,6 +248,20 @@
                                  const float* row_a, const float* col_a, const float* row_b, const float* col_b,
                                  float* loss_partials, float* wgrad_partials, int32_t n_part, void* stream);
 
+int32_t gd_del1_chain_fold_covers(int32_t n_sel, int32_t d, int32_t h);
+int gd_del1_chain_fold_loss_wgrad_f32(const float* a, int64_t ld_a, const int32_t* idx, int32_t n_sel, const float* w_fold,
+                                      const float* bias_fold, int32_t d, float* z, int64_t ld_z, uint32_t* sign_io,
+                                      const int32_t* loss_slot, const float* tm, const float* coef, const float* cnt_signed,
+                                      const float* dt, int64_t ld_dt, int32_t d_next, const float* w_next, float* loss_partials,
+                                      float* wgrad_partials_t, float* colsum_partials, int32_t n_part, void* stream);
+int gd_layer1_fold_f32(const float* w1, const float* b1, const float* wd, float* w_fold, float* bias_fold, void* stream);
+int gd_step_tail_fold1_f32(const float* partials1_t, const float* colsum1, int32_t n_part1, int32_t d1, int32_t accumulate1,
+                           const float* w1, const float* b1, float* dw1, float* param1, float* exp_avg1, float* exp_avg_sq1,
+                           float* w_fold, float* bias_fold, const float* partials2, int32_t n_part2, int32_t d2, int32_t accumulate2,
+                           float* dw2, float* param2, float* exp_avg2, float* exp_avg_sq2, double lr, double beta1, double beta2,
+                           double eps, const float* loss_partials1, int32_t n1, const float* loss_partials2, int32_t n2,
+                           float* hist, int32_t capacity, int32_t* pos, int32_t* iter, int32_t* arrive, void* stream);
+
 
 int64_t gd_rowpair_mse_workspace(int32_t n_seg);
 int gd_rowpair_mse_f32(const float* z, int64_t ld_z, const float* o, int64_t ld_o, int32_t d,
```

Result: faster. 2086 iters/s (median of 6 runs) (+7.7%).
